# GAP-LAB-CUHK-SZ/gaustudio

Hardware: AMD Instinct MI355X
Metric: Mpixels/s fwd+bwd @1M Gaussians 1920x1080 (higher is better)
Workload: dtype f32; 1 GPU; C3: 1M synthetic Gaussians, 1920x1080, SH degree 3, fwd+bwd (colour+depth+median+opacity consumed); gaussians=1000000, width=1920, height=1080, sh_degree=3, tiles=8160, views_per_rank=1, loss=colour + depth + median + opacity gradients consumed, camera=static (the same view every step), parallelism=single GPU

## Files before the change

### __graft_entry__.py

```python
import os
import subprocess
import sys

ROOT = os.path.dirname(os.path.abspath(__file__))
if ROOT not in sys.path:
    sys.path.insert(0, ROOT)


def build() -> None:
    subprocess.check_call(["make", "-C", os.path.join(ROOT, "gaustudio_amd", "csrc"), "-j4"])
    subprocess.check_call(["make", "-C", os.path.join(ROOT, "oracle"), "all"])
    ref_script = os.path.join(ROOT, "oracle", "build_ref.sh")
    if os.path.isdir("/root/reference") and os.path.exists(ref_script):
        subprocess.check_call(["bash", ref_script])
    import ctypes
    import gaustudio_amd
    import gaustudio_diff_gaussian_rasterization as g
    L = g._C.lib()
    assert L.gsr_abi_version() == 6
    for sym in ("gsr_forward", "gsr_backward", "gsr_mark_visible", "gsr_backward_scratch_bytes", "gsr_last_error",
                "gsr_inspect_geometry", "gsr_inspect_binning", "gsr_inspect_image", "gsr_inspect_backward_sums", "gsr_set_profiling",
                "gsr_last_forward_ms", "gsr_last_backward_ms", "gsr_forward_raw", "gsr_backward_raw", "gsr_forward_ex", "gsr_backward_ex", "gsr_options_init", "gsr_depth_to_points",
                "gsr_depth_to_normals", "gsr_depth_epilogue", "gsr_backward_parts", "gsr_set_option", "gsr_get_option", "gsr_selftest", "gsr_inspect_counts", "gsr_inspect_staged", "gsr_tsdf_integrate", "gsr_tsdf_integrate_map", "gsr_tsdf_export_blocks", "gsr_tsdf_mc_classify", "gsr_tsdf_mc_emit", "gsr_msg_header_words", "gsr_visible_index", "gsr_union_index", "gsr_pack_rows", "gsr_unpack_rows", "gsr_pack_geometry", "gsr_unpack_geometry",
                "gsr_sh_grad_from_packed", "gsr_band_classes", "gsr_mesh_rasterize", "gsr_mesh_interpolate",
                "gsr_mesh_vertex_normals", "gsr_mesh_visible_faces", "gsr_psr_rasterize", "gsr_psr_spectral", "gsr_psr_interp",
                "gsr_psr_normalize", "gsr_psr_mc_classify", "gsr_psr_mc_emit", "gsr_psr_mc_normals", "gsr_psr_rasterize_bwd",
                "gsr_psr_interp_bwd", "gsr_psr_spectral_bwd", "gsr_psr_normalize_bwd", "gsr_ctsdf_touch", "gsr_ctsdf_integrate",
                "gsr_ctsdf_export_blocks", "gsr_ctsdf_mc_classify", "gsr_ctsdf_mc_emit", "gsr_hull_pack_masks", "gsr_hull_carve",
                "gsr_voxel_plan", "gsr_voxel_count", "gsr_voxel_emit", "gsr_voxel_sort", "gsr_voxel_closest",
                "gsr_mesh_bake_select", "gsr_mesh_bake_sample", "gsr_mesh_seeds",
                "gsr_mean_dist3", "gsr_mean_dist3_ex", "gsr_point_seeds", "gsr_depth_seed_pack",
                "gsr_scaffold_count", "gsr_scaffold_emit", "gsr_scaffold_backward",
                "gsr_photometric_fwd", "gsr_photometric_bwd"):
        getattr(L, sym)
    for fn in ("rasterize_gaussians", "rasterize_gaussians_backward", "mark_visible"):
        assert callable(getattr(g._C.native(), fn))
    ctypes.CDLL(os.path.join(ROOT, "oracle", "liboracle.so"))
    ctypes.CDLL(os.path.join(ROOT, "oracle", "libtsdforacle.so"))


def smoke() -> None:
    import numpy as np
    import torch
    from gaustudio_amd import scenes
    from gaustudio_diff_gaussian_rasterization import GaussianRasterizationSettings, GaussianRasterizer
    from oracle import pyoracle as po

    assert torch.cuda.is_available(), "smoke() needs a ROCm GPU"
    dev = torch.device("cuda", 0)
    cam = scenes.make_camera(256, 160)
    sc = scenes.make_scene(5000, cam, seed=0, sigma_px_median=2.0)
    leaves = {k: getattr(sc, k).to(dev).requires_grad_(True) for k in ("means3D", "scales", "rotations", "opacities", "shs")}
    means2D = torch.zeros_like(leaves["means3D"], requires_grad=True)
    rs = GaussianRasterizationSettings(cam.height, cam.width, cam.tanfovx, cam.tanfovy, torch.zeros(3), 1.0,
                                       cam.viewmatrix.to(dev), cam.projmatrix.to(dev), 3, cam.campos.to(dev), False, False)
    import gaustudio_amd
    grads = scenes.make_output_grads(cam)
    out_default = GaussianRasterizer(rs)(means3D=leaves["means3D"], means2D=means2D, opacities=leaves["opacities"], shs=leaves["shs"],
                                         scales=leaves["scales"], rotations=leaves["rotations"])
    torch.autograd.backward([out_default[0], out_default[2], out_default[3], out_default[4]], [g.to(dev) for g in grads])
    torch.cuda.synchronize()
    grads_default = {k: v.grad.clone() for k, v in leaves.items()}
    for v in leaves.values():
        v.grad = None
    with gaustudio_amd.options(fast_exp=False):
        color, radii, depth, median, opac = GaussianRasterizer(rs)(
            means3D=leaves["means3D"], means2D=means2D, opacities=leaves["opacities"], shs=leaves["shs"],
            scales=leaves["scales"], rotations=leaves["rotations"])
        torch.autograd.backward([color, depth, median, opac], [g.to(dev) for g in grads])
    torch.cuda.synchronize()

    st = po.forward(sc.means3D.numpy(), sc.opacities.numpy(), cam.viewmatrix.numpy(), cam.projmatrix.numpy(),
                    cam.campos.numpy(), cam.width, cam.height, cam.tanfovx, cam.tanfovy, sh_degree=3,
                    shs=sc.shs.numpy(), scales=sc.scales.numpy(), rotations=sc.rotations.numpy())
    bw = po.backward(st, *[g.numpy() for g in grads])
    for name, a, b in (("color", color, st["color"]), ("depth", depth, st["depth"]), ("median", median, st["median"]),
                       ("opacity", opac, st["opacity"]), ("radii", radii, st["radii"])):
        assert np.array_equal(a.detach().cpu().numpy(), b), f"smoke: {name} differs from the oracle"
    for k, ok in dict(means3D="dL_dmeans3D", scales="dL_dscales", rotations="dL_drotations", opacities="dL_dopacity",
                      shs="dL_dsh").items():
        a = leaves[k].grad.cpu().numpy()
        b = bw[ok].reshape(a.shape)
        assert np.abs(a - b).max() <= 2e-4 * np.abs(b).max(), f"smoke: grad {k} off"
    sys.path.insert(0, os.path.join(ROOT, "tests"))
    import attribution
    ours = {k: out_default[i].detach().cpu().numpy() for k, i in (("color", 0), ("depth", 2), ("opacity", 4))}
    rep = attribution.attribute_images(st, cam.width, cam.height, {k: st[k] for k in ours}, ours, tol=1e-5, depth_scale=20.0)
    assert not rep["unattributed"], f"smoke (default mode): {len(rep['unattributed'])} of {rep['flagged']} pixels beyond 1e-5 are no threshold events"
    assert np.array_equal(out_default[1].cpu().numpy(), st["radii"])
    for k, ok in dict(means3D="dL_dmeans3D", scales="dL_dscales", rotations="dL_drotations", opacities="dL_dopacity", shs="dL_dsh").items():
        a = grads_default[k].cpu().numpy()
        b = bw[ok].reshape(a.shape)
        assert np.abs(a - b).max() <= 2e-4 * np.abs(b).max(), f"smoke (default mode): grad {k} off"
    print(f"smoke ok: R={st['num_rendered']}, reproducible mode bit-exact vs oracle, default (fast_exp) mode within 1e-5 "
          f"({rep['flagged']} pixel(s) beyond it, all attributed threshold events), "
          f"5 gradient tensors within 2e-4 of scale in both")


if __name__ == "__main__":
    build()
    print("build ok")
```

### gaustudio_amd/_C.py

```python
import ctypes
import os

import torch

from . import _abi

_HERE = os.path.dirname(os.path.abspath(__file__))
_LIB_PATH = os.path.join(_HERE, "libgsrast.so")
_lib = None


def lib():
    global _lib
    if _lib is None:
        if not os.path.exists(_LIB_PATH):
            raise ImportError(
                f"{_LIB_PATH} not found: the HIP extension is not built "
                "(run `python -c 'import __graft_entry__ as g; g.build()'` or `make -C gaustudio_amd/csrc`). "
                "gaustudio_amd has no CPU fallback.")
        L = ctypes.CDLL(_LIB_PATH)
        L.gsr_last_error.restype = ctypes.c_char_p
        L.gsr_backward_scratch_bytes.restype = ctypes.c_size_t
        L.gsr_backward_scratch_bytes.argtypes = [ctypes.c_int, ctypes.c_int]
        L.gsr_abi_version.restype = ctypes.c_int
# ... 109 lines not shown


def sh_grad_from_packed(means3D, campos, msgs, offsets, degree, out):
    _call("gsr_sh_grad_from_packed", out.device, out.shape[0], int(degree), out.shape[1], offsets.numel(), means3D, campos, msgs,
          offsets, out)
    return out


def set_grad_arena(outs, keys=(), sh_chunks=1, hook=None, colors_out=None, band_split=0, band_hook=None, class_hook=None):
    native().set_grad_arena(list(outs), [int(k) for k in keys], int(sh_chunks), hook, colors_out, int(band_split), band_hook, class_hook)


def band_classes(radii, geom_buffer, split_tile_row):
    P = int(radii.shape[0])
    first = torch.empty(P, dtype=torch.int32, device=radii.device)
    second = torch.empty(P, dtype=torch.int32, device=radii.device)
    _call("gsr_band_classes", radii.device, P, radii, geom_buffer, int(split_tile_row), first, second)
    return first, second


def set_option(name, value):
    L = lib()
    rc = L.gsr_set_option(name.encode(), ctypes.c_int(int(value)))
    if rc < 0:
        raise _err(L, rc)


def get_option(name):
    return int(lib().gsr_get_option(name.encode()))


def selftest(device=None):
    dev = torch.device("cuda", torch.cuda.current_device()) if device is None else torch.device(device)
    return _call("gsr_selftest", dev)


def inspect_counts(imgBuffer, width, height):
    out = (ctypes.c_uint32 * 4)()
    _call("gsr_inspect_counts", imgBuffer.device, imgBuffer, width, height, out)
    return dict(num_binned=int(out[0]), max_tile=int(out[1]), num_rendered=int(out[2]), overflow=int(out[3]))


def inspect_staged(imgBuffer, width, height):
    out = ctypes.c_ulonglong(0)
    _call("gsr_inspect_staged", imgBuffer.device, imgBuffer, int(width), int(height), ctypes.byref(out))
    return int(out.value)


def mark_visible(means3D, viewmatrix, projmatrix):
    return native().mark_visible(means3D, viewmatrix, projmatrix)



def inspect_geometry(geomBuffer, radii):
    dev = radii.device
    P = radii.numel()
    out = dict(means2D=torch.empty((P, 2), dtype=torch.float32, device=dev),
               depths=torch.empty((P,), dtype=torch.float32, device=dev),
               conic_opacity=torch.empty((P, 4), dtype=torch.float32, device=dev),
               rgb=torch.empty((P, 3), dtype=torch.float32, device=dev),
               clamped=torch.empty((P, 3), dtype=torch.uint8, device=dev),
               tiles_touched=torch.empty((P,), dtype=torch.int32, device=dev))
    _call("gsr_inspect_geometry", dev, geomBuffer, P, radii, *out.values())
    return out


def inspect_binning(binningBuffer, imgBuffer, R, width, height):
    dev = imgBuffer.device
    T = ((width + 15) // 16) * ((height + 15) // 16)
    point_list = torch.empty((max(int(R), 0),), dtype=torch.int32, device=dev)
    ranges = torch.empty((T, 2), dtype=torch.int32, device=dev)
    _call("gsr_inspect_binning", dev, binningBuffer, imgBuffer, int(R), width, height, point_list, ranges)
    return point_list, ranges


def inspect_image(imgBuffer, width, height):
    dev = imgBuffer.device
    final_T = torch.empty((height, width), dtype=torch.float32, device=dev)
    n_contrib = torch.empty((height, width), dtype=torch.int32, device=dev)
    _call("gsr_inspect_image", dev, imgBuffer, width, height, final_T, n_contrib)
    return final_T, n_contrib


def set_profiling(enable):
    lib().gsr_set_profiling(ctypes.c_int(int(enable)))


def last_forward_ms():
    a = (ctypes.c_float * 5)()
    n = lib().gsr_last_forward_ms(a)
    if not n:
        return None
    d = dict(zip(("preprocess", "scan", "scatter", "sort", "composite"), list(a)))
    d["calls"] = n
    return d


def last_backward_ms():
    a = (ctypes.c_float * 2)()
    n = lib().gsr_last_backward_ms(a)
    if not n:
        return None
    d = dict(zip(("composite_bwd", "preprocess_bwd"), list(a)))
    d["calls"] = n
    return d
```

### gaustudio_amd/csrc/gsr_api.hip

```cpp
#include "../../include/gsrast.h"
#include "gsr_internal.h"

#include <dlfcn.h>

#include <atomic>
#include <unordered_map>
#include <cstddef>
#include <cstdio>
#include <cstdlib>
#include <cstring>
#include <mutex>
#include <string>
#include <vector>

using namespace gsr;

namespace {

thread_local std::string g_err;
struct ProfSet {
	hipEvent_t ev[6];
	uint32_t have = 0;
};
struct ProfLog {
// ... 417 lines not shown
	hipStream_t s = (hipStream_t)stream;
	g_err.clear();
	if (P <= 0) return GSR_OK;
	if (!means3D || !viewmatrix || !present) return fail(GSR_ERR_ARG, "gsr_mark_visible: NULL argument", __FILE__, __LINE__);
	const float* view = viewmatrix;
	float* tmp = nullptr;
	if (!is_device_ptr(viewmatrix)) {
		HIP_TRY(hipMallocAsync((void**)&tmp, 16 * sizeof(float), s));
		HIP_TRY(hipMemcpyAsync(tmp, viewmatrix, 16 * sizeof(float), hipMemcpyHostToDevice, s));
		view = tmp;
	}
	launch_mark_visible(P, means3D, view, present, s);
	hipError_t e = hipGetLastError();
	if (tmp) (void)hipFreeAsync(tmp, s);
	if (e != hipSuccess) return fail(GSR_ERR_HIP, "mark_visible launch", __FILE__, __LINE__, e);
	return GSR_OK;
}

static int forward_impl(const gsr_options* opt, gsr_alloc_fn geometry_alloc, void* geometry_ctx, gsr_alloc_fn binning_alloc, void* binning_ctx,
                        gsr_alloc_fn image_alloc, void* image_ctx, int P, int D, int M, const float* background,
                        int width, int height, const float* means3D, const float* shs, const float* shs_rest,
                        const float* colors_precomp, const float* opacities, const float* scales, float scale_modifier,
                        const float* rotations, const float* cov3D_precomp, int activation_flags,
                        const float* viewmatrix, const float* projmatrix, const float* cam_pos, float tan_fovx,
                        float tan_fovy, int prefiltered, float* out_color, float* out_depth, float* out_median_depth,
                        float* out_opacity, int* radii, int debug, void* stream)
{
	hipStream_t s = (hipStream_t)stream;
	g_err.clear();
	if (width <= 0 || height <= 0) return fail(GSR_ERR_ARG, "gsr_forward: bad image size", __FILE__, __LINE__);
	if (!out_color || !out_depth || !out_median_depth || !out_opacity)
		return fail(GSR_ERR_ARG, "gsr_forward: NULL output", __FILE__, __LINE__);
	const size_t HW = (size_t)width * height;
	if (P <= 0) {
		hipLaunchKernelGGL(fill_empty_outputs_kernel, dim3((unsigned)((HW + 255) / 256)), dim3(256), 0, s, HW,
		                   out_color, out_depth, out_median_depth, out_opacity);
		STAGE_CHECK("fill_empty_outputs", debug, s);
		return 0;
	}
	if (!means3D || !opacities || !viewmatrix || !projmatrix || !cam_pos || !radii)
		return fail(GSR_ERR_ARG, "gsr_forward: NULL required input", __FILE__, __LINE__);
	if (!colors_precomp && !shs)
		return fail(GSR_ERR_ARG, "For non-RGB, provide precomputed Gaussian colors!", __FILE__, __LINE__);
	if (!cov3D_precomp && (!scales || !rotations))
		return fail(GSR_ERR_ARG, "gsr_forward: need scales+rotations or cov3D_precomp", __FILE__, __LINE__);
	if (!colors_precomp && (D < 0 || D > 3 || (D + 1) * (D + 1) > M))
		return fail(GSR_ERR_ARG, "gsr_forward: SH degree does not fit the stored coefficients", __FILE__, __LINE__);
	if (!geometry_alloc || !binning_alloc || !image_alloc)
		return fail(GSR_ERR_ARG, "gsr_forward: NULL allocator", __FILE__, __LINE__);

	{
		const int rc = check_sticky("gsr_forward");
		if (rc < 0) return rc;
	}
	Resolved ro = resolve_options(opt);
#ifndef GSR_AB_VARIANTS
	if (ro.fwd_variant == 1)
		return fail(GSR_ERR_ARG, "gsr_forward: fwd_variant 1 (the per-wave A/B kernel) is not in this build (make AB=1; gsr_get_option(\"ab_variants\"))", __FILE__, __LINE__);
#endif
	if (ro.fast_exp && ro.fwd_variant == 1) {
		if (ro.fast_exp_explicit)
			return fail(GSR_ERR_ARG, "gsr_forward: fast_exp needs the per-quarter compositing kernels (fwd_variant 0)", __FILE__, __LINE__);
		ro.fast_exp = 0;
	}
	const GeomLayout gl((size_t)P);
	const ImgLayout il(width, height);
	if (il.gx > 65535 || il.gy > 65535) return fail(GSR_ERR_ARG, "gsr_forward: image too large", __FILE__, __LINE__);
	char* geom = geometry_alloc(geometry_ctx, gl.total);
	const bool lds_bin = bin_lds_path_ok(il.T);
	const size_t hm_off = il.total;
	char* img = image_alloc(image_ctx, il.total + (lds_bin ? align_up(bin_hist_bytes(P, il.T)) : 0));
	if (!geom || !img) return fail(GSR_ERR_ALLOC, "gsr_forward: allocator returned NULL", __FILE__, __LINE__);

	remember_forward_mode(img, ro.fast_exp != 0, ro.forward_only);

	GsCam* cam = reinterpret_cast<GsCam*>(geom + gl.cam);
	GsRec* recs = reinterpret_cast<GsRec*>(geom + gl.recs);
	GsCtl* ctl = reinterpret_cast<GsCtl*>(img + il.ctl);
	uint2* ranges = reinterpret_cast<uint2*>(img + il.ranges);
	uint32_t* tile_count = reinterpret_cast<uint32_t*>(img + il.tile_count);
	float* final_T = reinterpret_cast<float*>(img + il.final_T);
	uint32_t* n_contrib = reinterpret_cast<uint32_t*>(img + il.n_contrib);
	uint32_t* med_pos = reinterpret_cast<uint32_t*>(img + il.med_pos);

	Timer tm(prof_next(g_fwd_log), s, kFwdStages, g_prof_fwd_mask);
	static_assert(sizeof(GsCtl) == 8 * sizeof(uint32_t), "stage_cam_kernel clears GsCtl word by word");
	if (!lds_bin) HIP_TRY(hipMemsetAsync(img + il.ctl, 0, il.final_T - il.ctl, s));
	{
		const float* const src[4] = {viewmatrix, projmatrix, cam_pos, background};
		float* const dst[4] = {cam->view, cam->proj, cam->campos, cam->bg};
		const int n[4] = {16, 16, 3, 3};
		const bool banded = ro.band_hi > 0 || ro.band_lo > 0;
		const uint32_t word = (ro.fast_exp ? GSR_CTL_OPT_FAST_EXP : 0u) | (ro.tight ? GSR_CTL_OPT_TIGHT : 0u) |
		                      (ro.cull ? GSR_CTL_OPT_CULL : 0u) | (ro.fwd_variant == 1 ? GSR_CTL_OPT_WAVE_LISTS : 0u) |
		                      (banded ? GSR_CTL_OPT_BAND : 0u) | (ro.forward_only ? GSR_CTL_OPT_FORWARD_ONLY : 0u);
		HIP_TRY(stage_small(src, dst, n, s, &ctl->opts, word, reinterpret_cast<uint32_t*>(ctl), 8));
	}

	FwdArgs a;
	a.P = P; a.D = D; a.M = M; a.W = width; a.H = height;
	a.means3D = means3D; a.shs = shs; a.colors_precomp = colors_precomp; a.opacities = opacities;
	a.scales = scales; a.scale_modifier = scale_modifier; a.rotations = rotations; a.cov3D_precomp = cov3D_precomp;
	a.tan_fovx = tan_fovx; a.tan_fovy = tan_fovy; a.prefiltered = prefiltered;
	a.shs_rest = shs_rest; a.act = activation_flags;
	a.tight = ro.tight != 0;
	a.band_lo = ro.band_lo > 0 ? ro.band_lo : 0;
	a.band_hi = ro.band_hi;

	tm.mark();
	uint32_t* tiles_touched = reinterpret_cast<uint32_t*>(geom + gl.tiles_touched);
	uint32_t* bsums = reinterpret_cast<uint32_t*>(geom + gl.bsums);
	uint32_t* refsums = reinterpret_cast<uint32_t*>(geom + gl.refsums);
	uint32_t* Hm = reinterpret_cast<uint32_t*>(img + hm_off);
	uint4* binfo_w = reinterpret_cast<uint4*>(geom + gl.binfo);
	const uint4* binfo = (lds_bin && g_opt_bininfo.load() != 0) ? binfo_w : nullptr;
	launch_preprocess_fwd(a, cam, il, radii, recs, ro.forward_only ? nullptr : reinterpret_cast<float*>(geom + gl.shjac), binfo_w, tiles_touched, bsums, refsums,
	                      lds_bin ? nullptr : tile_count, ctl, s);
	STAGE_CHECK("preprocess_fwd", debug, s);
	tm.mark();
	if (lds_bin) {
		launch_bin_hist(P, il.gx, il.T, tiles_touched, recs, binfo, Hm, tile_count, s);
		STAGE_CHECK("bin_hist", debug, s);
	}
	GsCtl* host = pinned_ctl();
	if (!host) return fail(GSR_ERR_HIP, "hipHostMalloc", __FILE__, __LINE__);
	launch_tile_scan(il.T, tile_count, ranges, (int)gl.nblk, bsums, refsums, ctl, host, s);
	STAGE_CHECK("tile_scan", debug, s);
	hipEvent_t ev = readback_event();
	if (ev) HIP_TRY(hipEventRecord(ev, s));
	uint32_t* goff = reinterpret_cast<uint32_t*>(geom + gl.goff);
	bool goff_done = false;
	tm.mark();

	DevState& ds = dev_state();
	const bool nocull = ro.cull == 0;
	const bool wave_lists = ro.fwd_variant == 1;
	bool skew_now = g_opt_tile_order.load() != 0 && ds.skew.load() != 0;
	auto launch_rest = [&](uint32_t cap, int long_level) -> int {
		const bool with_long = long_level > 0;
		const BinLayout bl((size_t)cap, with_long, il.T);
		char* bin = binning_alloc(binning_ctx, bl.total);
		if (!bin) return fail(GSR_ERR_ALLOC, "gsr_forward: binning allocator returned NULL", __FILE__, __LINE__);
		uint64_t* keys = reinterpret_cast<uint64_t*>(bin + bl.keys);
		uint64_t* keys2 = reinterpret_cast<uint64_t*>(bin + bl.keys2);
		uint32_t* point_list = reinterpret_cast<uint32_t*>(bin + bl.point_list);
		if (cap > 0) {
			if (lds_bin) {
				launch_bin_scatter2(P, il.gx, il.T, tiles_touched, recs, binfo, Hm, ranges, keys, bsums, goff, ctl, cap, s);
				goff_done = true;
			}
			else
				launch_bin_scatter(P, il.gx, radii, tiles_touched, recs, ranges, tile_count, keys, ctl, cap, s);
			STAGE_CHECK("bin_scatter", debug, s);
		}
		if (!goff_done) {
			launch_goff_apply(P, tiles_touched, bsums, goff, s);
			STAGE_CHECK("goff_apply", debug, s);
			goff_done = true;
		}
		tm.mark();
		if (cap > 0) {
			launch_tile_sort(il.T, true, long_level, ranges, keys, keys2, point_list, bin + bl.queue, (size_t)cap, ctl, cap, long_level > 0 ? sticky_word() : nullptr, s);
			STAGE_CHECK("tile_sort", debug, s);
		}
		tm.mark();
		const uint32_t* order = nullptr;
		if (skew_now && cap > 0) {
			uint32_t* o = reinterpret_cast<uint32_t*>(img + il.tile_order);
			launch_tile_order_fwd(il.T, ranges, o, ctl, cap, s);
			order = o;
		}
		launch_composite_fwd(il, width, height, ranges, point_list, recs, out_color, out_depth, out_median_depth,
		                     out_opacity, final_T, n_contrib, med_pos, ctl, cap,
		                     long_level >= 2 ? 0xffffffffu : (long_level == 1 ? GSR_SORT_GIANT : GSR_SORT_LDS_MAX), nocull, wave_lists, ro.fast_exp != 0, order,
		                     tile_count , s);
		STAGE_CHECK("composite_fwd", debug, s);
		tm.mark();
		return 0;
	};

	const uint32_t cap0 = ds.cap.load();
	const int long0 = ds.long_lists.load();
	const bool speculate = !debug && ro.speculative != 0 && cap0 > 0;
	if (speculate) {
		const int rc = launch_rest(cap0, long0);
		if (rc < 0) return rc;
	}
	if (ev) HIP_TRY(hipEventSynchronize(ev));
	else HIP_TRY(hipStreamSynchronize(s));
	const uint32_t Rb = host->num_binned, max_tile = host->max_tile_count;
	if (host->err_prefiltered)
		return fail(GSR_ERR_PREFILTERED, "Point is filtered although prefiltered is set. This shouldn't happen!",
		            __FILE__, __LINE__);
	if ((host->err_overflow & 1u) || host->ref_rendered > 0x7fffffffu || Rb > 0x7fffffffu)
		return fail(GSR_ERR_ARG, "gsr_forward: more than 2^31 - 1 (tile, Gaussian) instances", __FILE__, __LINE__);
	const int need_long = max_tile > GSR_SORT_GIANT ? 2 : (max_tile > GSR_SORT_LDS_MAX ? 1 : 0);
	if (!speculate || Rb > cap0 || need_long > long0) {
		const int rc = launch_rest(Rb, need_long);
		if (rc < 0) return rc;
	}
	const uint32_t want = Rb + Rb / 4 + 4096u;
	uint32_t cur = ds.cap.load();
	for (;;) {
		const uint32_t next = cur < want ? want : (cur - (cur - want) / 8 > want + 4096u ? cur - (cur - want) / 8 : want);
		if (next == cur || ds.cap.compare_exchange_weak(cur, next)) break;
	}
	ds.long_lists.store(need_long);
	if (debug) {
		GsCtl c;
		HIP_TRY(hipMemcpyAsync(&c, img + il.ctl, sizeof(GsCtl), hipMemcpyDeviceToHost, s));
		HIP_TRY(hipStreamSynchronize(s));
		if (c.err_overflow & 2u)
			return fail(GSR_ERR_HIP, "gsr_forward: the long-list sort overflowed a work queue (SortQueueLayout bound violated)", __FILE__, __LINE__);
	}
	const int skew = (g_opt_tile_order.load() != 0 && max_tile > GSR_SORT_LDS_MAX && (uint64_t)max_tile * (uint64_t)il.T > 4ull * Rb) ? 1 : 0;
	remember_forward_skew(img, skew);
	ds.skew.store(skew);
	return (int)host->ref_rendered;
}

int gsr_forward(gsr_alloc_fn geometry_alloc, void* geometry_ctx, gsr_alloc_fn binning_alloc, void* binning_ctx,
                gsr_alloc_fn image_alloc, void* image_ctx, int P, int D, int M, const float* background, int width,
                int height, const float* means3D, const float* shs, const float* colors_precomp,
                const float* opacities, const float* scales, float scale_modifier, const float* rotations,
                const float* cov3D_precomp, const float* viewmatrix, const float* projmatrix, const float* cam_pos,
                float tan_fovx, float tan_fovy, int prefiltered, float* out_color, float* out_depth,
                float* out_median_depth, float* out_opacity, int* radii, int debug, void* stream)
{
	return forward_impl(nullptr, geometry_alloc, geometry_ctx, binning_alloc, binning_ctx, image_alloc, image_ctx, P, D, M,
	                    background, width, height, means3D, shs, nullptr, colors_precomp, opacities, scales,
	                    scale_modifier, rotations, cov3D_precomp, 0, viewmatrix, projmatrix, cam_pos, tan_fovx, tan_fovy,
	                    prefiltered, out_color, out_depth, out_median_depth, out_opacity, radii, debug, stream);
}

int gsr_forward_raw(gsr_alloc_fn geometry_alloc, void* geometry_ctx, gsr_alloc_fn binning_alloc, void* binning_ctx,
                    gsr_alloc_fn image_alloc, void* image_ctx, int P, int D, int M, const float* background, int width,
                    int height, const float* means3D, const float* f_dc, const float* f_rest, const float* raw_opacities,
                    const float* raw_scales, float scale_modifier, const float* raw_rotations, int activation_flags,
                    const float* viewmatrix, const float* projmatrix, const float* cam_pos, float tan_fovx,
                    float tan_fovy, int prefiltered, float* out_color, float* out_depth, float* out_median_depth,
                    float* out_opacity, int* radii, int debug, void* stream)
{
	if (P > 0 && (!f_dc || (M > 1 && !f_rest) || !raw_scales || !raw_rotations))
		return fail(GSR_ERR_ARG, "gsr_forward_raw: f_dc, f_rest, raw_scales and raw_rotations are required", __FILE__, __LINE__);
	return forward_impl(nullptr, geometry_alloc, geometry_ctx, binning_alloc, binning_ctx, image_alloc, image_ctx, P, D, M,
	                    background, width, height, means3D, f_dc, M > 1 ? f_rest : nullptr, nullptr, raw_opacities,
	                    raw_scales, scale_modifier, raw_rotations, nullptr, activation_flags, viewmatrix, projmatrix, cam_pos,
	                    tan_fovx, tan_fovy, prefiltered, out_color, out_depth, out_median_depth, out_opacity, radii, debug,
	                    stream);
}

int gsr_forward_ex(const gsr_options* opt, gsr_alloc_fn geometry_alloc, void* geometry_ctx, gsr_alloc_fn binning_alloc,
                   void* binning_ctx, gsr_alloc_fn image_alloc, void* image_ctx, int P, int D, int M,
                   const float* background, int width, int height, const float* means3D, const float* shs,
                   const float* shs_rest, const float* colors_precomp, const float* opacities, const float* scales,
                   float scale_modifier, const float* rotations, const float* cov3D_precomp, int activation_flags,
                   const float* viewmatrix, const float* projmatrix, const float* cam_pos, float tan_fovx, float tan_fovy,
                   int prefiltered, float* out_color, float* out_depth, float* out_median_depth, float* out_opacity,
                   int* radii, int debug, void* stream)
{
	return forward_impl(opt, geometry_alloc, geometry_ctx, binning_alloc, binning_ctx, image_alloc, image_ctx, P, D, M,
	                    background, width, height, means3D, shs, shs_rest, colors_precomp, opacities, scales, scale_modifier,
	                    rotations, cov3D_precomp, activation_flags, viewmatrix, projmatrix, cam_pos, tan_fovx, tan_fovy,
	                    prefiltered, out_color, out_depth, out_median_depth, out_opacity, radii, debug, stream);
}

size_t gsr_geometry_bytes(int P) { return GeomLayout((size_t)(P > 0 ? P : 0)).total; }
size_t gsr_image_bytes(int width, int height) { return (width > 0 && height > 0) ? ImgLayout(width, height).total : 0; }

size_t gsr_backward_scratch_bytes(int P, int R)
{
	return BwdLayout((size_t)(P > 0 ? P : 0), (size_t)(R > 0 ? R : 0)).total;
}

static int bwd_variant(int opt, hipStream_t s)
{
	if (opt >= 0) return opt;
	DevState& ds = dev_state();
	int st = ds.selftest.load();
	if (st < 0) {
		st = gsr_selftest((void*)s);
		if (st < 0) st = 0;
		ds.selftest.store(st);
	}
	return (st & 3) == 3 ? 0 : 1;
}

static int backward_impl(const gsr_options* opt, int parts, int sh_g0, int sh_g1, int P, int D, int M, int R, const float* background, int width, int height,
                         const float* means3D, const float* shs, const float* shs_rest, const float* colors_precomp,
                         const float* scales, float scale_modifier, const float* rotations, const float* cov3D_precomp,
                         int activation_flags, float tan_fovx, float tan_fovy, const int* radii, const char* geom_buffer,
                         const char* binning_buffer, const char* image_buffer, const float* dL_dpix,
                         const float* dL_dpix_depth, const float* dL_dpix_median_depth,
                         const float* dL_dpix_final_opacity, float* dL_dmean2D, float* dL_dopacity, float* dL_dcolor,
                         float* dL_dmean3D, float* dL_dcov3D, float* dL_dsh, float* dL_dsh_rest, float* dL_dscale,
                         float* dL_drot, char* scratch, int debug, void* stream)
{
	hipStream_t s = (hipStream_t)stream;
	g_err.clear();
	if (P <= 0) return GSR_OK;
	if (!geom_buffer || !image_buffer || !binning_buffer || !scratch || !radii || !means3D)
		return fail(GSR_ERR_ARG, "gsr_backward: NULL buffer", __FILE__, __LINE__);
	const bool sh_colors = (parts & GSR_BWD_PART_SH_COLORS) != 0;
	const int colors_early = ((parts & GSR_BWD_PART_COLORS_EARLY) && sh_colors) ? GSR_PART_COLORS_EARLY : 0;
	if (!dL_dmean2D || !dL_dopacity || !dL_dcolor || !dL_dmean3D || (!dL_dcov3D && cov3D_precomp) || !dL_dscale || !dL_drot ||
	    (M > 0 && !dL_dsh && !sh_colors))
		return fail(GSR_ERR_ARG, "gsr_backward: NULL output", __FILE__, __LINE__);
	if (sh_colors && (!shs || shs_rest || colors_precomp))
		return fail(GSR_ERR_ARG, "gsr_backward: GSR_BWD_PART_SH_COLORS needs SH colours in one [P,M,3] tensor", __FILE__, __LINE__);
	if (shs && (D < 0 || D > 3 || (D + 1) * (D + 1) > M))
		return fail(GSR_ERR_ARG, "gsr_backward: SH degree does not fit the stored coefficients", __FILE__, __LINE__);

	const GeomLayout gl((size_t)P);
	const ImgLayout il(width, height);
	const BinLayout bl((size_t)(R > 0 ? R : 0));
	const GsCam* cam = reinterpret_cast<const GsCam*>(geom_buffer + gl.cam);
	const GsRec* recs = reinterpret_cast<const GsRec*>(geom_buffer + gl.recs);
	const uint2* ranges = reinterpret_cast<const uint2*>(image_buffer + il.ranges);
	const float* final_T = reinterpret_cast<const float*>(image_buffer + il.final_T);
	const uint32_t* n_contrib = reinterpret_cast<const uint32_t*>(image_buffer + il.n_contrib);
	const uint32_t* med_pos = reinterpret_cast<const uint32_t*>(image_buffer + il.med_pos);
	const uint32_t* point_list = reinterpret_cast<const uint32_t*>(binning_buffer + bl.point_list);
	const BwdLayout wl((size_t)P, (size_t)(R > 0 ? R : 0));
	const uint32_t* goff = reinterpret_cast<const uint32_t*>(geom_buffer + gl.goff);
	const uint32_t* clampw = reinterpret_cast<const uint32_t*>(geom_buffer + gl.binfo) + 2;
	float* bg_dev = reinterpret_cast<float*>(scratch + wl.bg);
	float* rows = reinterpret_cast<float*>(scratch + wl.rows);
	uint8_t* row_flags = reinterpret_cast<uint8_t*>(scratch + wl.flags);

	const int band_phase = (parts & GSR_BWD_PART_BAND_FIRST) ? 0 : ((parts & GSR_BWD_PART_BAND_SECOND) ? 1 : -1);
	int band_split = 0;
	if (band_phase >= 0) {
		if ((parts & GSR_BWD_PART_BAND_FIRST) && (parts & GSR_BWD_PART_BAND_SECOND))
			return fail(GSR_ERR_ARG, "gsr_backward: GSR_BWD_PART_BAND_FIRST and _SECOND are two calls", __FILE__, __LINE__);
		if (!(parts & GSR_BWD_PART_MAIN) || (parts & GSR_BWD_PART_SH))
			return fail(GSR_ERR_ARG, "gsr_backward: a band call runs GSR_BWD_PART_MAIN only (the SH stage follows the second band as its own call)", __FILE__, __LINE__);
		band_split = sh_g0 < 0 ? 0 : (sh_g0 > il.gy ? il.gy : sh_g0);
	}
	BwdArgs a;
	a.cls_mode = band_phase + 1;
	a.cls_split = band_split;
	a.P = P; a.D = D; a.M = M; a.W = width; a.H = height;
	a.means3D = means3D; a.shs = shs; a.colors_precomp = colors_precomp; a.scales = scales;
	a.scale_modifier = scale_modifier; a.rotations = rotations; a.cov3D_precomp = cov3D_precomp;
	a.tan_fovx = tan_fovx; a.tan_fovy = tan_fovy; a.radii = radii;
	a.shs_rest = shs_rest; a.act = activation_flags;

	FwdMode fwd;
	{
		int rc = check_sticky("gsr_backward");
		if (rc < 0) return rc;
		rc = lookup_forward(image_buffer, il.ctl, s, &fwd);
		if (rc < 0) return rc;
	}
	if (fwd.forward_only)
		return fail(GSR_ERR_ARG, "gsr_backward: these buffers come from a forward_only forward (gsr_options.forward_only): it kept nothing for a backward", __FILE__, __LINE__);
	if (debug) {
		GsCtl c;
		HIP_TRY(hipMemcpyAsync(&c, image_buffer + il.ctl, sizeof(GsCtl), hipMemcpyDeviceToHost, s));
		HIP_TRY(hipStreamSynchronize(s));
		if (c.opts & GSR_CTL_OPT_FORWARD_ONLY)
			return fail(GSR_ERR_ARG, "gsr_backward: these buffers come from a forward_only forward (gsr_options.forward_only): it kept nothing for a backward", __FILE__, __LINE__);
		if (c.err_overflow & 2u)
			return fail(GSR_ERR_HIP, "gsr_backward: the forward's long-list sort overflowed a work queue (point_list is not sorted)", __FILE__, __LINE__);
	}
	if (!(parts & GSR_BWD_PART_MAIN)) {
		launch_preprocess_bwd(a, cam, recs, clampw, reinterpret_cast<const float*>(geom_buffer + gl.shjac), goff, rows, nullptr, dL_dmean2D, dL_dopacity, dL_dcolor, dL_dmean3D, dL_dcov3D,
		                      dL_dsh, dL_dsh_rest, dL_dscale, dL_drot, GSR_PART_SH | (sh_colors ? GSR_PART_SH_COLORS : 0) | colors_early, sh_g0, sh_g1, s);
		STAGE_CHECK("preprocess_bwd_sh", debug, s);
		return GSR_OK;
	}

	Timer tm(prof_next(g_bwd_log), s, kBwdStages, g_prof_bwd_mask);
	const bool flagged = (size_t)(R > 0 ? R : 0) > (size_t)il.T * GSR_FLAG_AVG;
	GsBg bgv;
	bgv.dptr = (background != nullptr && is_device_ptr(background)) ? background : nullptr;
	for (int i = 0; i < 3; i++) bgv.host[i] = (background != nullptr && bgv.dptr == nullptr) ? background[i] : 0.f;
	bgv.flag_dst = reinterpret_cast<uint32_t*>(bg_dev + 8);
	bgv.flag = flagged ? 1u : 0u;
	bgv.tile_order = nullptr;
	bgv.tile_lo = band_phase == 1 ? (uint32_t)band_split * (uint32_t)il.gx : 0u;
	bgv.tile_hi = band_phase == 0 ? (uint32_t)band_split * (uint32_t)il.gx : 0xffffffffu;
	if (R <= 0) {
		const float* const src[4] = {nullptr, nullptr, nullptr, nullptr};
		float* const dst[4] = {nullptr, nullptr, nullptr, nullptr};
		const int n[4] = {0, 0, 0, 0};
		HIP_TRY(stage_small(src, dst, n, s, bgv.flag_dst, bgv.flag));
	}
	if (flagged) {
		if (band_phase != 1) HIP_TRY(hipMemsetAsync(row_flags, 0, (size_t)R, s));
	} else
		row_flags = nullptr;

	tm.mark();
	if (R > 0) {
		Resolved ro = resolve_options(opt);
		{
			const int fwd_mode = fwd.fast_exp;
			if (!ro.fast_exp_explicit) ro.fast_exp = fwd_mode;
			if (fwd_mode != (ro.fast_exp != 0))
				return fail(GSR_ERR_ARG, "gsr_backward: fast_exp differs from the forward that produced these buffers", __FILE__, __LINE__);
		}
		if (debug) {
			GsCtl c;
			HIP_TRY(hipMemcpyAsync(&c, image_buffer + il.ctl, sizeof(GsCtl), hipMemcpyDeviceToHost, s));
			HIP_TRY(hipStreamSynchronize(s));
			if (!ro.fast_exp_explicit) ro.fast_exp = (c.opts & GSR_CTL_OPT_FAST_EXP) ? 1 : 0;
			if (((c.opts & GSR_CTL_OPT_FAST_EXP) != 0u) != (ro.fast_exp != 0))
				return fail(GSR_ERR_ARG, "gsr_backward: fast_exp differs from the forward that produced these buffers", __FILE__, __LINE__);
		}
		int variant = bwd_variant(ro.bwd_variant, s);
#ifndef GSR_AB_VARIANTS
		if (variant & 2)
			return fail(GSR_ERR_ARG, "gsr_backward: bwd_variant bit 1 (the per-wave A/B kernel) is not in this build (make AB=1; gsr_get_option(\"ab_variants\"))", __FILE__, __LINE__);
#endif
		if (ro.fast_exp) {
			if (variant & 2) return fail(GSR_ERR_ARG, "gsr_backward: fast_exp needs the per-quarter kernel (bwd_variant bit 1 clear)", __FILE__, __LINE__);
			variant |= 8;
		}
		if (fwd.skew) {
			uint32_t* tw = reinterpret_cast<uint32_t*>(const_cast<char*>(image_buffer) + il.tile_work);
			uint32_t* to = reinterpret_cast<uint32_t*>(const_cast<char*>(image_buffer) + il.tile_order);
			launch_tile_order(il.T, n_contrib, tw, to, s);
			bgv.tile_order = to;
		}
		launch_composite_bwd(il, width, height, bgv, ranges, point_list, recs, goff, final_T, n_contrib, med_pos, dL_dpix,
		                     dL_dpix_depth, dL_dpix_median_depth, dL_dpix_final_opacity, rows, row_flags,
		                     reinterpret_cast<const GsCtl*>(image_buffer + il.ctl), variant, s);
		STAGE_CHECK("composite_bwd", debug, s);
	}
	tm.mark();
	launch_preprocess_bwd(a, cam, recs, clampw, reinterpret_cast<const float*>(geom_buffer + gl.shjac), goff, rows, row_flags, dL_dmean2D, dL_dopacity, dL_dcolor, dL_dmean3D, dL_dcov3D, dL_dsh,
	                      dL_dsh_rest, dL_dscale, dL_drot,
	                      GSR_PART_GEOM | ((parts & GSR_BWD_PART_SH) ? GSR_PART_SH : 0) | (sh_colors ? GSR_PART_SH_COLORS : 0) | colors_early,
	                      sh_g0, sh_g1, s);
	STAGE_CHECK("preprocess_bwd", debug, s);
	tm.mark();
	return GSR_OK;
}

int gsr_backward(int P, int D, int M, int R, const float* background, int width, int height, const float* means3D,
                 const float* shs, const float* colors_precomp, const float* scales, float scale_modifier,
                 const float* rotations, const float* cov3D_precomp, const float* viewmatrix,
                 const float* projmatrix, const float* campos, float tan_fovx, float tan_fovy, const int* radii,
                 const char* geom_buffer, const char* binning_buffer, const char* image_buffer,
                 const float* dL_dpix, const float* dL_dpix_depth, const float* dL_dpix_median_depth,
                 const float* dL_dpix_final_opacity, float* dL_dmean2D, float* dL_dopacity, float* dL_dcolor,
                 float* dL_dmean3D, float* dL_dcov3D, float* dL_dsh, float* dL_dscale, float* dL_drot,
                 char* scratch, int debug, void* stream)
{
	(void)viewmatrix; (void)projmatrix; (void)campos;
	return backward_impl(nullptr, GSR_BWD_PART_MAIN | GSR_BWD_PART_SH, 0, P, P, D, M, R, background, width, height, means3D, shs, nullptr, colors_precomp, scales,
	                     scale_modifier, rotations, cov3D_precomp, 0, tan_fovx, tan_fovy, radii, geom_buffer,
	                     binning_buffer, image_buffer, dL_dpix, dL_dpix_depth, dL_dpix_median_depth,
	                     dL_dpix_final_opacity, dL_dmean2D, dL_dopacity, dL_dcolor, dL_dmean3D, dL_dcov3D, dL_dsh,
	                     nullptr, dL_dscale, dL_drot, scratch, debug, stream);
}

int gsr_backward_parts(int parts, int sh_g0, int sh_g1, int P, int D, int M, int R, const float* background, int width,
                       int height, const float* means3D, const float* shs, const float* colors_precomp, const float* scales,
                       float scale_modifier, const float* rotations, const float* cov3D_precomp, float tan_fovx,
                       float tan_fovy, const int* radii, const char* geom_buffer, const char* binning_buffer,
                       const char* image_buffer, const float* dL_dpix, const float* dL_dpix_depth,
                       const float* dL_dpix_median_depth, const float* dL_dpix_final_opacity, float* dL_dmean2D,
                       float* dL_dopacity, float* dL_dcolor, float* dL_dmean3D, float* dL_dcov3D, float* dL_dsh,
                       float* dL_dscale, float* dL_drot, char* scratch, int debug, void* stream)
{
	if (!(parts & (GSR_BWD_PART_MAIN | GSR_BWD_PART_SH)))
		return fail(GSR_ERR_ARG, "gsr_backward_parts: nothing to do", __FILE__, __LINE__);
	if ((parts & GSR_BWD_PART_SH) && sh_g0 % 256 != 0)
		return fail(GSR_ERR_ARG, "gsr_backward_parts: sh_g0 must be a multiple of 256", __FILE__, __LINE__);
	return backward_impl(nullptr, parts, sh_g0, sh_g1, P, D, M, R, background, width, height, means3D, shs, nullptr, colors_precomp,
	                     scales, scale_modifier, rotations, cov3D_precomp, 0, tan_fovx, tan_fovy, radii, geom_buffer,
	                     binning_buffer, image_buffer, dL_dpix, dL_dpix_depth, dL_dpix_median_depth,
	                     dL_dpix_final_opacity, dL_dmean2D, dL_dopacity, dL_dcolor, dL_dmean3D, dL_dcov3D, dL_dsh,
	                     nullptr, dL_dscale, dL_drot, scratch, debug, stream);
}

int gsr_backward_ex(const gsr_options* opt, int parts, int sh_g0, int sh_g1, int P, int D, int M, int R,
                    const float* background, int width, int height, const float* means3D, const float* shs,
                    const float* shs_rest, const float* colors_precomp, const float* scales, float scale_modifier,
                    const float* rotations, const float* cov3D_precomp, int activation_flags, float tan_fovx,
                    float tan_fovy, const int* radii, const char* geom_buffer, const char* binning_buffer,
                    const char* image_buffer, const float* dL_dpix, const float* dL_dpix_depth,
                    const float* dL_dpix_median_depth, const float* dL_dpix_final_opacity, float* dL_dmean2D,
                    float* dL_dopacity, float* dL_dcolor, float* dL_dmean3D, float* dL_dcov3D, float* dL_dsh,
                    float* dL_dsh_rest, float* dL_dscale, float* dL_drot, char* scratch, int debug, void* stream)
{
	if (!(parts & (GSR_BWD_PART_MAIN | GSR_BWD_PART_SH)))
		return fail(GSR_ERR_ARG, "gsr_backward_ex: nothing to do", __FILE__, __LINE__);
	if ((parts & GSR_BWD_PART_SH) && !(parts & (GSR_BWD_PART_BAND_FIRST | GSR_BWD_PART_BAND_SECOND)) && sh_g0 % 256 != 0)
		return fail(GSR_ERR_ARG, "gsr_backward_ex: sh_g0 must be a multiple of 256", __FILE__, __LINE__);
	return backward_impl(opt, parts, sh_g0, sh_g1, P, D, M, R, background, width, height, means3D, shs, shs_rest,
	                     colors_precomp, scales, scale_modifier, rotations, cov3D_precomp, activation_flags, tan_fovx, tan_fovy,
	                     radii, geom_buffer, binning_buffer, image_buffer, dL_dpix, dL_dpix_depth, dL_dpix_median_depth,
	                     dL_dpix_final_opacity, dL_dmean2D, dL_dopacity, dL_dcolor, dL_dmean3D, dL_dcov3D, dL_dsh, dL_dsh_rest,
	                     dL_dscale, dL_drot, scratch, debug, stream);
}

int gsr_band_classes(int P, const int* radii, const char* geom_buffer, int split_tile_row, int* first, int* second, void* stream)
{
	g_err.clear();
	if (P <= 0) return GSR_OK;
	if (!radii || !geom_buffer) return fail(GSR_ERR_ARG, "gsr_band_classes: NULL argument", __FILE__, __LINE__);
	const GeomLayout gl((size_t)P);
	launch_band_classes(P, radii, reinterpret_cast<const GsRec*>(geom_buffer + gl.recs), split_tile_row, first, second, (hipStream_t)stream);
	STAGE_CHECK("band_classes", 0, (hipStream_t)stream);
	return GSR_OK;
}
// ... 134 lines not shown
int gsr_backward_raw(int P, int D, int M, int R, const float* background, int width, int height, const float* means3D,
                     const float* f_dc, const float* f_rest, const float* raw_scales, float scale_modifier,
                     const float* raw_rotations, int activation_flags, float tan_fovx, float tan_fovy,
                     const int* radii, const char* geom_buffer, const char* binning_buffer, const char* image_buffer,
                     const float* dL_dpix, const float* dL_dpix_depth, const float* dL_dpix_median_depth,
                     const float* dL_dpix_final_opacity, float* dL_dmean2D, float* dL_draw_opacity, float* dL_dcolor,
                     float* dL_dmean3D, float* dL_dcov3D, float* dL_df_dc, float* dL_df_rest, float* dL_draw_scale,
                     float* dL_draw_rot, char* scratch, int debug, void* stream)
{
	if (P > 0 && (!f_dc || (M > 1 && (!f_rest || !dL_df_rest)) || !dL_df_dc))
		return fail(GSR_ERR_ARG, "gsr_backward_raw: f_dc / f_rest and their gradient outputs are required", __FILE__, __LINE__);
	return backward_impl(nullptr, GSR_BWD_PART_MAIN | GSR_BWD_PART_SH, 0, P, P, D, M, R, background, width, height, means3D, f_dc, M > 1 ? f_rest : nullptr, nullptr, raw_scales,
	                     scale_modifier, raw_rotations, nullptr, activation_flags, tan_fovx, tan_fovy, radii, geom_buffer,
	                     binning_buffer, image_buffer, dL_dpix, dL_dpix_depth, dL_dpix_median_depth,
	                     dL_dpix_final_opacity, dL_dmean2D, dL_draw_opacity, dL_dcolor, dL_dmean3D, dL_dcov3D, dL_df_dc,
	                     M > 1 ? dL_df_rest : nullptr, dL_draw_scale, dL_draw_rot, scratch, debug, stream);
}

int gsr_inspect_geometry(const char* geom_buffer, int P, const int* radii, float* means2D, float* depths,
                         float* conic_opacity, float* rgb, unsigned char* clamped, uint32_t* tiles_touched,
                         void* stream)
{
	hipStream_t s = (hipStream_t)stream;
	g_err.clear();
	if (P <= 0) return GSR_OK;
	if (!geom_buffer || !radii) return fail(GSR_ERR_ARG, "gsr_inspect_geometry: NULL buffer", __FILE__, __LINE__);
	const GeomLayout gl((size_t)P);
	hipLaunchKernelGGL(inspect_geometry_kernel, dim3((P + 255) / 256), dim3(256), 0, s, P, radii,
	                   reinterpret_cast<const GsRec*>(geom_buffer + gl.recs),
	                   reinterpret_cast<const uint32_t*>(geom_buffer + gl.tiles_touched), means2D, depths, conic_opacity, rgb,
	                   clamped, tiles_touched);
	STAGE_CHECK("inspect_geometry", 0, s);
	return GSR_OK;
}

int gsr_inspect_backward_sums(const char* geom_buffer, const char* scratch, int P, int R, const int* radii,
                               float* sums, void* stream)
{
	hipStream_t s = (hipStream_t)stream;
	g_err.clear();
	if (P <= 0) return GSR_OK;
	if (!geom_buffer || !scratch || !radii || !sums)
		return fail(GSR_ERR_ARG, "gsr_inspect_backward_sums: NULL argument", __FILE__, __LINE__);
	const GeomLayout gl((size_t)P);
	const BwdLayout wl((size_t)P, (size_t)(R > 0 ? R : 0));
	uint32_t flagged = 0;
	HIP_TRY(hipMemcpyAsync(&flagged, scratch + wl.bg + 8 * sizeof(float), sizeof(uint32_t), hipMemcpyDeviceToHost, s));
	HIP_TRY(hipStreamSynchronize(s));
	launch_inspect_sums(P, radii, reinterpret_cast<const GsRec*>(geom_buffer + gl.recs),
	                    reinterpret_cast<const uint32_t*>(geom_buffer + gl.goff),
	                    reinterpret_cast<const float*>(scratch + wl.rows), flagged ? reinterpret_cast<const uint8_t*>(scratch + wl.flags) : nullptr,
	                    sums, s);
	STAGE_CHECK("inspect_backward_sums", 0, s);
	return GSR_OK;
}

int gsr_inspect_binning(const char* binning_buffer, const char* image_buffer, int R, int width, int height,
                        uint32_t* point_list, uint32_t* ranges, void* stream)
{
	hipStream_t s = (hipStream_t)stream;
	g_err.clear();
	if (!image_buffer) return fail(GSR_ERR_ARG, "gsr_inspect_binning: NULL buffer", __FILE__, __LINE__);
	const ImgLayout il(width, height);
	const BinLayout bl((size_t)(R > 0 ? R : 0));
	if (ranges) HIP_TRY(hipMemcpyAsync(ranges, image_buffer + il.ranges, sizeof(uint2) * (size_t)il.T, hipMemcpyDeviceToDevice, s));
	if (point_list && R > 0) {
		if (!binning_buffer) return fail(GSR_ERR_ARG, "gsr_inspect_binning: NULL binning buffer", __FILE__, __LINE__);
		HIP_TRY(hipMemcpyAsync(point_list, binning_buffer + bl.point_list, sizeof(uint32_t) * (size_t)R, hipMemcpyDeviceToDevice, s));
	}
	return GSR_OK;
}

int gsr_inspect_image(const char* image_buffer, int width, int height, float* final_T, uint32_t* n_contrib,
                      void* stream)
{
	hipStream_t s = (hipStream_t)stream;
	g_err.clear();
	if (!image_buffer) return fail(GSR_ERR_ARG, "gsr_inspect_image: NULL buffer", __FILE__, __LINE__);
	const ImgLayout il(width, height);
	hipLaunchKernelGGL(inspect_image_kernel, dim3(il.T), dim3(256), 0, s, il.gx, width, height,
	                   reinterpret_cast<const float*>(image_buffer + il.final_T),
	                   reinterpret_cast<const uint32_t*>(image_buffer + il.n_contrib), final_T, n_contrib);
	STAGE_CHECK("inspect_image", 0, s);
	return GSR_OK;
}

int gsr_surfel_forward(const gsr_options* opt, gsr_alloc_fn geometry_alloc, void* geometry_ctx, gsr_alloc_fn binning_alloc,
                       void* binning_ctx, gsr_alloc_fn image_alloc, void* image_ctx, int P, int D, int M, const float* background,
                       int width, int height, const float* means3D, const float* shs, const float* colors_precomp,
                       const float* opacities, const float* scales, float scale_modifier, const float* rotations,
                       const float* viewmatrix, const float* projmatrix, const float* cam_pos, float* out_color, float* out_allmap,
                       int* radii, int debug, void* stream)
{
	hipStream_t s = (hipStream_t)stream;
	g_err.clear();
	if (width <= 0 || height <= 0) return fail(GSR_ERR_ARG, "gsr_surfel_forward: bad image size", __FILE__, __LINE__);
	if (!out_color || !out_allmap) return fail(GSR_ERR_ARG, "gsr_surfel_forward: NULL output", __FILE__, __LINE__);
	if (!geometry_alloc || !binning_alloc || !image_alloc)
		return fail(GSR_ERR_ARG, "gsr_surfel_forward: NULL allocator", __FILE__, __LINE__);
	const size_t HW = (size_t)width * height;
	if (P <= 0) {
		HIP_TRY(hipMemsetAsync(out_color, 0, sizeof(float) * 3 * HW, s));
		HIP_TRY(hipMemsetAsync(out_allmap, 0, sizeof(float) * 7 * HW, s));
		return 0;
	}
	if (!means3D || !opacities || !scales || !rotations || !viewmatrix || !projmatrix || !cam_pos || !radii)
		return fail(GSR_ERR_ARG, "gsr_surfel_forward: NULL required input", __FILE__, __LINE__);
	if ((colors_precomp != nullptr) == (shs != nullptr))
		return fail(GSR_ERR_ARG, "gsr_surfel_forward: provide exactly one of SHs or precomputed colours", __FILE__, __LINE__);
	if (!colors_precomp && (D < 0 || D > 3 || (D + 1) * (D + 1) > M))
		return fail(GSR_ERR_ARG, "gsr_surfel_forward: SH degree does not fit the stored coefficients", __FILE__, __LINE__);
	{
		const int rc = check_sticky("gsr_surfel_forward");
		if (rc < 0) return rc;
	}
	const Resolved ro = resolve_options(opt);
	const SurfGeomLayout gl((size_t)P);
	const ImgLayout il0(width, height);
	if (!bin_lds_path_ok(il0.T))
		return fail(GSR_ERR_ARG, "gsr_surfel_forward: image too large (the surfel path bins through the LDS tile histogram only)", __FILE__, __LINE__);
	const SurfImgLayout sl(width, height, bin_hist_bytes(P, il0.T));
	const ImgLayout& il = sl.il;
	char* geom = geometry_alloc(geometry_ctx, gl.total);
	char* img = image_alloc(image_ctx, sl.total);
	if (!geom || !img) return fail(GSR_ERR_ALLOC, "gsr_surfel_forward: allocator returned NULL", __FILE__, __LINE__);
	remember_forward_mode(img, ro.fast_exp != 0, 0);

	GsCam* cam = reinterpret_cast<GsCam*>(geom + gl.cam);
	SurfRec* recs = reinterpret_cast<SurfRec*>(geom + gl.recs);
	uint32_t* tiles_touched = reinterpret_cast<uint32_t*>(geom + gl.tiles_touched);
	uint32_t* goff = reinterpret_cast<uint32_t*>(geom + gl.goff);
	uint32_t* bsums = reinterpret_cast<uint32_t*>(geom + gl.bsums);
	uint32_t* refsums = reinterpret_cast<uint32_t*>(geom + gl.refsums);
	uint4* binfo = reinterpret_cast<uint4*>(geom + gl.binfo);
	GsCtl* ctl = reinterpret_cast<GsCtl*>(img + il.ctl);
	uint2* ranges = reinterpret_cast<uint2*>(img + il.ranges);
	uint32_t* tile_count = reinterpret_cast<uint32_t*>(img + il.tile_count);
	uint32_t* Hm = reinterpret_cast<uint32_t*>(img + sl.hist);
	{
		const float* const src[4] = {viewmatrix, projmatrix, cam_pos, background};
		float* const dst[4] = {cam->view, cam->proj, cam->campos, cam->bg};
		const int n[4] = {16, 16, 3, 3};
		HIP_TRY(stage_small(src, dst, n, s, &ctl->opts, ro.fast_exp ? GSR_CTL_OPT_FAST_EXP : 0u, reinterpret_cast<uint32_t*>(ctl), 8));
	}
	SurfFwdArgs a;
	a.P = P; a.D = D; a.M = M; a.W = width; a.H = height;
	a.means3D = means3D; a.shs = shs; a.colors_precomp = colors_precomp; a.opacities = opacities;
	a.scales = scales; a.scale_modifier = scale_modifier; a.rotations = rotations;
	launch_surfel_preprocess_fwd(a, cam, il, radii, recs, reinterpret_cast<float*>(geom + gl.shjac), binfo, tiles_touched, bsums, refsums, s);
	STAGE_CHECK("surfel_preprocess_fwd", debug, s);
	launch_bin_hist(P, il.gx, il.T, tiles_touched, nullptr, binfo, Hm, tile_count, s);
	STAGE_CHECK("bin_hist", debug, s);
	GsCtl* host = pinned_ctl();
	if (!host) return fail(GSR_ERR_HIP, "hipHostMalloc", __FILE__, __LINE__);
	launch_tile_scan(il.T, tile_count, ranges, (int)gl.nblk, bsums, refsums, ctl, host, s);
	STAGE_CHECK("tile_scan", debug, s);
	hipEvent_t ev = readback_event();
	if (ev) {
		HIP_TRY(hipEventRecord(ev, s));
		HIP_TRY(hipEventSynchronize(ev));
	} else
		HIP_TRY(hipStreamSynchronize(s));
	const uint32_t R = host->num_binned, max_tile = host->max_tile_count;
	if ((host->err_overflow & 1u) || host->ref_rendered > 0x7fffffffu || R > 0x7fffffffu)
		return fail(GSR_ERR_ARG, "gsr_surfel_forward: more than 2^31 - 1 (tile, surfel) instances", __FILE__, __LINE__);
	const int long_level = max_tile > GSR_SORT_GIANT ? 2 : (max_tile > GSR_SORT_LDS_MAX ? 1 : 0);
// ... 95 lines not shown
```

### gaustudio_amd/csrc/gsr_internal.h

```cpp
#pragma once
#include "gsr_common.h"
#include <stddef.h>

namespace gsr {

static inline size_t align_up(size_t v, size_t a = 256) { return (v + a - 1) / a * a; }

#define GSR_PRE_BLOCK 256
struct GeomLayout {
	size_t cam, recs, tiles_touched, goff, bsums, refsums, shjac, binfo, total;
	size_t nblk;
	explicit GeomLayout(size_t P)
	{
		nblk = (P + GSR_PRE_BLOCK - 1) / GSR_PRE_BLOCK;
		cam = 0;
		recs = align_up(sizeof(GsCam));
		tiles_touched = recs + align_up(sizeof(GsRec) * P);
		goff = tiles_touched + align_up(sizeof(uint32_t) * P);
		bsums = goff + align_up(sizeof(uint32_t) * (P + 1));
		refsums = bsums + align_up(sizeof(uint32_t) * (nblk + 1));
		shjac = refsums + align_up(sizeof(uint32_t) * (nblk + 1));
		binfo = shjac + align_up(sizeof(float) * 9 * P);
		total = binfo + align_up(sizeof(uint4) * P);
	}
};

struct ImgLayout {
	size_t ctl, ranges, tile_count, final_T, n_contrib, med_pos, tile_work, tile_order, total;
	int gx, gy, T;
	ImgLayout(int W, int H)
	{
		gx = (W + GSR_BLOCK_X - 1) / GSR_BLOCK_X;
		gy = (H + GSR_BLOCK_Y - 1) / GSR_BLOCK_Y;
		T = gx * gy;
		ctl = 0;
		ranges = align_up(sizeof(GsCtl));
		tile_count = ranges + align_up(sizeof(uint2) * (size_t)T);
		final_T = tile_count + align_up(sizeof(uint32_t) * (size_t)T);
		n_contrib = final_T + align_up(sizeof(float) * (size_t)T * GSR_TILE_PIX);
		med_pos = n_contrib + align_up(sizeof(uint32_t) * (size_t)T * GSR_TILE_PIX);
		tile_work = med_pos + align_up(sizeof(uint32_t) * (size_t)T * GSR_TILE_PIX);
		tile_order = tile_work + align_up(sizeof(uint32_t) * (size_t)T);
		total = tile_order + align_up(sizeof(uint32_t) * (size_t)T);
	}
};

size_t sort_queue_bytes(size_t R, int T);
struct BinLayout {
	size_t point_list, keys, keys2, queue, total;
	explicit BinLayout(size_t R, bool with_tmp = false, int T = 0)
	{
		point_list = 0;
		keys = align_up(sizeof(uint32_t) * R);
		keys2 = keys + align_up(sizeof(uint64_t) * R);
		queue = keys2 + align_up(sizeof(uint64_t) * R);
		total = with_tmp ? queue + align_up(sort_queue_bytes(R, T)) : keys2;
		if (total == 0) total = 256;
	}
};
#define GSR_SORT_LDS_MAX 1024u

struct FwdArgs {
	int P, D, M, W, H;
	const float* means3D;
	const float* shs;
	const float* colors_precomp;
	const float* opacities;
	const float* scales;
	float scale_modifier;
	const float* rotations;
	const float* cov3D_precomp;
	float tan_fovx, tan_fovy;
	int prefiltered;
	const float* shs_rest;
	int act;
	int tight;
	int band_lo, band_hi;
};

void launch_mark_visible(int P, const float* means3D, const float* view, unsigned char* present, hipStream_t s);
void launch_preprocess_fwd(const FwdArgs& a, const GsCam* cam, const ImgLayout& il, int* radii, GsRec* recs, float* shjac, uint4* binfo,
                           uint32_t* tiles_touched, uint32_t* bsums, uint32_t* refsums, uint32_t* tile_count,
                           GsCtl* ctl, hipStream_t s);
void launch_tile_scan(int T, uint32_t* tile_count, uint2* ranges, int nblk, uint32_t* bsums, const uint32_t* refsums,
                      GsCtl* ctl, GsCtl* host_ctl, hipStream_t s);
void launch_goff_apply(int P, const uint32_t* tiles_touched, const uint32_t* bsums, uint32_t* goff, hipStream_t s);
void launch_bin_scatter(int P, int gx, const int* radii, const uint32_t* tiles_touched, const GsRec* recs,
                        const uint2* ranges, uint32_t* cursor, uint64_t* keys, const GsCtl* ctl, uint32_t cap,
                        hipStream_t s);
int bin_chunks(int P, int T);
size_t bin_hist_bytes(int P, int T);
bool bin_lds_path_ok(int T);
void launch_bin_hist(int P, int gx, int T, const uint32_t* tiles_touched, const GsRec* recs, const uint4* binfo, uint32_t* Hm,
                     uint32_t* tile_count, hipStream_t s);
void launch_bin_scatter2(int P, int gx, int T, const uint32_t* tiles_touched, const GsRec* recs, const uint4* binfo, uint32_t* Hm,
                         const uint2* ranges, uint64_t* keys, const uint32_t* bsums, uint32_t* goff, const GsCtl* ctl, uint32_t cap, hipStream_t s);
#define GSR_PART_REGS 8192u
#define GSR_SORT_MANY 1024u
#ifndef GSR_SORT_GIANT
#define GSR_SORT_GIANT 8192u
#endif
void launch_tile_sort(int T, bool with_short, int long_level, const uint2* ranges, uint64_t* keys, uint64_t* keys2,
                      uint32_t* point_list, char* queue, size_t R, GsCtl* ctl, uint32_t cap, uint32_t* host_err, hipStream_t s);
void launch_composite_fwd(const ImgLayout& il, int W, int H, const uint2* ranges, const uint32_t* point_list,
                          const GsRec* recs, float* out_color, float* out_depth, float* out_median,
                          float* out_opacity, float* final_T, uint32_t* n_contrib, uint32_t* med_pos, GsCtl* ctl, uint32_t cap, uint32_t max_sorted, bool nocull, bool wave_lists, bool fast_exp,
                          const uint32_t* tile_order, uint32_t* staged_out, hipStream_t s);
void launch_tile_order_fwd(int T, const uint2* ranges, uint32_t* order, const GsCtl* ctl, uint32_t cap, hipStream_t s);

struct BwdArgs {
	int P, D, M, W, H;
	const float* means3D;
	const float* shs;
	const float* colors_precomp;
	const float* scales;
	float scale_modifier;
	const float* rotations;
	const float* cov3D_precomp;
	float tan_fovx, tan_fovy;
	const int* radii;
	const float* shs_rest;
	int act;
	int cls_mode = 0, cls_split = 0;
};
#define GSR_ROW_STRIDE 12
#define GSR_FLAG_AVG 1024
#ifndef GSR_SUM_SLAB
#define GSR_SUM_SLAB 96
#endif
struct BwdLayout {
	size_t bg, flags, rows, total;
	BwdLayout(size_t P, size_t R)
	{
		(void)P;
		bg = 0;
		flags = bg + 256;
		rows = flags + align_up(R > 0 ? R : 1);
		total = rows + align_up(sizeof(float) * GSR_ROW_STRIDE * (R > 0 ? R : 1));
	}
};
struct GsBg {
	const float* dptr;
	float host[3];
	uint32_t* flag_dst;
	uint32_t flag;
	const uint32_t* tile_order;
	uint32_t tile_lo, tile_hi;
};
void launch_band_classes(int P, const int* radii, const GsRec* recs, int split, int* first, int* second, hipStream_t s);
void launch_tile_order(int T, const uint32_t* n_contrib, uint32_t* tile_work, uint32_t* tile_order, hipStream_t s);
void launch_composite_bwd(const ImgLayout& il, int W, int H, const GsBg& bg, const uint2* ranges,
                          const uint32_t* point_list, const GsRec* recs, const uint32_t* goff, const float* final_T,
                          const uint32_t* n_contrib, const uint32_t* med_pos, const float* dL_dpix, const float* dL_dpix_depth,
                          const float* dL_dpix_median, const float* dL_dpix_opacity, float* rows, uint8_t* row_flags,
                          const GsCtl* ctl, int variant, hipStream_t s);
#define GSR_PART_GEOM 1
#define GSR_PART_SH 2
#define GSR_PART_SH_COLORS 4
#define GSR_PART_COLORS_EARLY 8
void launch_preprocess_bwd(const BwdArgs& a, const GsCam* cam, const GsRec* recs, const uint32_t* clampw, const float* shjac, const uint32_t* goff,
                           const float* rows, const uint8_t* row_flags, float* dL_dmean2D, float* dL_dopacity, float* dL_dcolor,
                           float* dL_dmean3D, float* dL_dcov3D, float* dL_dsh, float* dL_dsh_rest, float* dL_dscale,
                           float* dL_drot, int parts, int sh_g0, int sh_g1, hipStream_t s);
void launch_bwd_selftest(const float* in, uint32_t* out, hipStream_t s);
void launch_sh_grad_from_colors(int P, int D, int M, int N, const float* means3D, const float* campos, const float* colors,
                                const uint32_t* msgs, const unsigned long long* msg_off, uint32_t hdr_words, float* dL_dsh, hipStream_t s);
void launch_inspect_sums(int P, const int* radii, const GsRec* recs, const uint32_t* goff, const float* rows,
                         const uint8_t* row_flags,
                         float* sums10, hipStream_t s);

struct __attribute__((aligned(16))) SurfRec {
	float4 q0, q1, q2, q3, q4;
};
static_assert(sizeof(SurfRec) == 80, "SurfRec must be 80 bytes");
struct SurfGeomLayout {
	size_t cam, recs, tiles_touched, goff, bsums, refsums, shjac, binfo, total;
	size_t nblk;
	explicit SurfGeomLayout(size_t P)
	{
		nblk = (P + GSR_PRE_BLOCK - 1) / GSR_PRE_BLOCK;
		cam = 0;
		recs = align_up(sizeof(GsCam));
		tiles_touched = recs + align_up(sizeof(SurfRec) * P);
		goff = tiles_touched + align_up(sizeof(uint32_t) * P);
		bsums = goff + align_up(sizeof(uint32_t) * (P + 1));
		refsums = bsums + align_up(sizeof(uint32_t) * (nblk + 1));
		shjac = refsums + align_up(sizeof(uint32_t) * (nblk + 1));
		binfo = shjac + align_up(sizeof(float) * 9 * P);
		total = binfo + align_up(sizeof(uint4) * P);
	}
};
struct SurfImgLayout {
	ImgLayout il;
	size_t m1, m2, m0, hist, total;
	SurfImgLayout(int W, int H, size_t hist_bytes) : il(W, H)
	{
		m1 = il.total;
		m2 = m1 + align_up(sizeof(float) * (size_t)il.T * GSR_TILE_PIX);
		m0 = m2 + align_up(sizeof(float) * (size_t)il.T * GSR_TILE_PIX);
		hist = m0 + align_up(sizeof(float) * (size_t)il.T * GSR_TILE_PIX);
		total = hist + align_up(hist_bytes > 0 ? hist_bytes : 1);
	}
};
#define GSR_SURF_ROW 16
struct SurfFwdArgs {
	int P, D, M, W, H;
	const float* means3D;
	const float* shs;
	const float* colors_precomp;
	const float* opacities;
	const float* scales;
	float scale_modifier;
	const float* rotations;
};
void launch_surfel_preprocess_fwd(const SurfFwdArgs& a, const GsCam* cam, const ImgLayout& il, int* radii, SurfRec* recs, float* shjac,
                                  uint4* binfo, uint32_t* tiles_touched, uint32_t* bsums, uint32_t* refsums, hipStream_t s);
void launch_surfel_composite_fwd(const ImgLayout& il, int W, int H, const uint2* ranges, const uint32_t* point_list, const SurfRec* recs,
                                 const GsCam* cam, float* out_color, float* out_allmap, float* final_T, uint32_t* n_contrib,
                                 uint32_t* med_pos, float* m1, float* m2, float* m0, bool fast_exp, hipStream_t s);
void launch_surfel_composite_bwd(const ImgLayout& il, int W, int H, const uint2* ranges, const uint32_t* point_list, const SurfRec* recs,
                                 const uint4* binfo, const uint32_t* goff, const float* final_T,
                                 const uint32_t* n_contrib, const uint32_t* med_pos, const float* m1, const float* m2, const float* m0,
                                 const GsCam* cam, const float* dL_dcolor, const float* dL_dallmap,
                                 float* rows, bool fast_exp, hipStream_t s);
void launch_surfel_preprocess_bwd(int P, int W, int H, const float* means3D, const float* scales, float scale_modifier,
                                  const float* rotations, const int* radii, const GsCam* cam, const SurfRec* recs,
                                  const uint32_t* goff, const float* rows, float* dL_dmean2D, float* dL_dopacity, float* dL_dcolor,
                                  float* dL_dmean3D, float* dL_dscale, float* dL_drot, hipStream_t s);

}
```

### gaustudio_amd/csrc/gsr_kernels_bwd.hip

```cpp
#include "gsr_internal.h"
#include "gsr_bwd_timing.h"

namespace gsr {

__device__ __constant__ float bSH_C0 = 0.28209479177387814f;
__device__ __constant__ float bSH_C1 = 0.4886025119029199f;
__device__ __constant__ float bSH_C2[5] = {1.0925484305920792f, -1.0925484305920792f, 0.31539156525252005f,
                                            -1.0925484305920792f, 0.5462742152960396f};
__device__ __constant__ float bSH_C3[7] = {-0.5900435899266435f, 2.890611442640554f, -0.4570457994644658f,
                                            0.3731763325901154f, -0.4570457994644658f, 1.445305721320277f,
                                            -0.5900435899266435f};

#define GSR_DPP_ADD(v, ctrl) v += __int_as_float(__builtin_amdgcn_update_dpp(0, __float_as_int(v), ctrl, 0xF, 0xF, true))
#define GSR_DPP_OF(v, ctrl) __int_as_float(__builtin_amdgcn_update_dpp(0, __float_as_int(v), ctrl, 0xF, 0xF, true))
__device__ __forceinline__ float half_swap_sum(float a, float b)
{
	const auto t = __builtin_amdgcn_permlane32_swap(__float_as_uint(a), __float_as_uint(b), false, false);
	return __uint_as_float(t[0]) + __uint_as_float(t[1]);
}
__device__ __forceinline__ float row_swap_sum(float p, float q)
{
	const auto t = __builtin_amdgcn_permlane16_swap(__float_as_uint(p), __float_as_uint(q), false, false);
	return __uint_as_float(t[0]) + __uint_as_float(t[1]);
}
// ... 55 lines not shown
			a_[0] += v0.x; a_[1] += v0.y; a_[2] += v0.z; a_[3] += v0.w; a_[4] += v1.x; a_[5] += v1.y;
			a_[6] += v1.z; a_[7] += v1.w; a_[8] += v2.x; a_[9] += v2.y;
		}
	}
	gs_sum_long_rows(b, e, rows, row_flags, lane, a_);
	if (idx >= P) return;
#pragma unroll
	for (int i = 0; i < 10; i++) out[10 * (size_t)idx + i] = a_[i];
}

void launch_inspect_sums(int P, const int* radii, const GsRec* recs, const uint32_t* goff, const float* rows,
                         const uint8_t* row_flags, float* sums10, hipStream_t s)
{
	hipLaunchKernelGGL(inspect_sums_kernel, dim3((P + 255) / 256), dim3(256), 0, s, P, radii, recs, goff, rows, row_flags,
	                   sums10);
}

#define GSR_BWD_THREADS 256
#define GSR_BWD_BATCH 64
#ifndef GSR_BWD_UNITS
#define GSR_BWD_UNITS 8
#endif
#define GSR_SLAB_STRIDE 65
#define GSR_PLANE_STRIDE 10
#define GSR_TAB_ROW 17

#ifdef GSR_AB_VARIANTS
__device__ __forceinline__ void gs_bwd_phase2(const int n, const float2* __restrict__ slab, const unsigned long long unit_js,
                                              const float4* __restrict__ sA, const float4* __restrict__ tab, const float fbx,
                                              const float fby, const int top, float* __restrict__ plane, const int lane)
{
	constexpr int NG = 64 / GSR_BWD_UNITS;
	constexpr int PPL = GSR_BWD_UNITS;
	const int u = lane & (GSR_BWD_UNITS - 1), g = lane / GSR_BWD_UNITS;
	const bool act = u < n;
	const int j = act ? (int)((unit_js >> (8 * u)) & 0xffull) : 0;
	const float2 ctr = *reinterpret_cast<const float2*>(&sA[j]);
	const uint32_t pos1 = (uint32_t)(top - j);
	const int prow = NG == 8 ? g : (g >> 1), pcol0 = NG == 8 ? 0 : ((g & 1) << 2);
	const float dy = ctr.y - (fby + (float)prow);
	const float X = ctr.x - (fbx + (float)pcol0);
	const float2* row = slab + u * GSR_SLAB_STRIDE + prow * 8 + pcol0;
	const float4* trow = tab + prow * GSR_TAB_ROW + 2 * pcol0;
	float S0 = 0.f, a0 = 0.f, a2 = 0.f, a5 = 0.f, a6 = 0.f, a7 = 0.f, a8 = 0.f, a9 = 0.f;
#pragma unroll
	for (int sx = 0; sx < PPL; sx++) {
		const float2 v = row[sx];
		const float4 c0 = trow[2 * sx], c1 = trow[2 * sx + 1];
		const float dx = X - (float)sx;
		const float t = v.x * dx;
		S0 += v.x;
		a0 += t;
		a2 = FMA(t, dx, a2);
		a5 = FMA(v.y, c1.x, a5);
		a6 = FMA(v.y, c0.x, a6);
		a7 = FMA(v.y, c0.y, a7);
		a8 = FMA(v.y, c0.z, a8);
		a9 = FMA(v.y, c0.w, a9) + ((__float_as_uint(c1.z) == pos1) ? c1.y : 0.f);
	}
	a5 += S0;
	const float a1 = dy * S0, a3 = dy * a0, a4 = dy * a1;
	const float r0 = half_swap_sum(a0, a1);
	const float r1 = half_swap_sum(a2, a3);
	const float r2 = half_swap_sum(a4, a5);
	const float r3 = half_swap_sum(a6, a7);
	const float r4 = half_swap_sum(a8, a9);
	float s0 = row_swap_sum(r0, r1), s1 = row_swap_sum(r2, r3), s2 = row_swap_sum(r4, 0.f);
	GSR_DPP_ADD(s0, 0x128); GSR_DPP_ADD(s1, 0x128); GSR_DPP_ADD(s2, 0x128);
	if (NG == 16) { GSR_DPP_ADD(s0, 0x124); GSR_DPP_ADD(s1, 0x124); GSR_DPP_ADD(s2, 0x124); }
	if (act && (lane & (16 - GSR_BWD_UNITS) & 15) == 0) {
		const int rw = lane >> 4;
		float* dst = plane + j * GSR_PLANE_STRIDE + (((rw & 1) << 1) | (rw >> 1));
		dst[0] = s0;
		dst[4] = s1;
		if ((rw & 1) == 0) dst[8] = s2;
	}
}

template <bool FLAGS, bool TSEL>
__global__ __launch_bounds__(GSR_BWD_THREADS) void composite_bwd_kernel(
    int T, int chunk, int gx, int W, int H, const GsBg bgv, const uint2* __restrict__ ranges,
    const uint32_t* __restrict__ point_list, const GsRec* __restrict__ recs, const uint32_t* __restrict__ goff,
    const float* __restrict__ final_T, const uint32_t* __restrict__ n_contrib, const uint32_t* __restrict__ med_pos,
    const float* __restrict__ dL_dpix, const float* __restrict__ dL_dpix_depth, const float* __restrict__ dL_dpix_median,
    const float* __restrict__ dL_dpix_opacity, float* __restrict__ rows, uint8_t* __restrict__ row_flags,
    const GsCtl* __restrict__ ctl)
{
	__shared__ float4 sA[GSR_BWD_BATCH];
	__shared__ float4 sB[GSR_BWD_BATCH];
	__shared__ float4 sC[GSR_BWD_BATCH];
	__shared__ uint32_t s_row[GSR_BWD_BATCH];
	__shared__ __attribute__((aligned(16))) float s_plane[4][GSR_BWD_BATCH * GSR_PLANE_STRIDE];
	__shared__ float2 s_slab[4][GSR_BWD_UNITS * GSR_SLAB_STRIDE];
	__shared__ float4 s_tab[4][8 * GSR_TAB_ROW];
	__shared__ int s_max[4];
	if (blockIdx.x == 0 && threadIdx.x == 0 && bgv.flag_dst != nullptr) *bgv.flag_dst = bgv.flag;
	const int tb_lo = (int)bgv.tile_lo, tb_n = (int)min(bgv.tile_hi, (uint32_t)T) - tb_lo;
	const int local = (blockIdx.x & 7) * chunk + (blockIdx.x >> 3);
	const int tile = bgv.tile_order ? ((int)blockIdx.x < T ? (int)bgv.tile_order[blockIdx.x] : T) : tb_lo + local;
	if ((!bgv.tile_order && ((int)(blockIdx.x >> 3) >= chunk || local >= tb_n)) || tile >= T) return;
	if ((uint32_t)tile < bgv.tile_lo || (uint32_t)tile >= bgv.tile_hi) return;
	const int tid = threadIdx.x;
	const int lane = tid & 63, wv = tid >> 6;
	const int tx = tile % gx, ty = tile / gx;
	int lx, ly;
	gs_pixel_of_thread(tid, lx, ly);
	const int px = tx * GSR_BLOCK_X + lx, py = ty * GSR_BLOCK_Y + ly;
	const bool inside = px < W && py < H;
	const float pixfx = (float)px, pixfy = (float)py;
	const float fbx = (float)(tx * GSR_BLOCK_X + ((wv & 1) << 3)), fby = (float)(ty * GSR_BLOCK_Y + ((wv >> 1) << 3));
	const float bx1 = fminf(fbx + 7.f, (float)(W - 1)), by1 = fminf(fby + 7.f, (float)(H - 1));
	const uint2 range = ranges[tile];

	const size_t sidx = (size_t)tile * GSR_TILE_PIX + tid;
	const float T_final = inside ? final_T[sidx] : 0.f;
	const int lc = inside ? (int)n_contrib[sidx] : 0;
	float dLp0 = 0.f, dLp1 = 0.f, dLp2 = 0.f, dLd = 0.f, dLo = 0.f;
	{
		float dLm = 0.f;
		uint32_t mpos = 0u;
		if (inside) {
			const size_t HW = (size_t)H * W;
			const size_t pix_id = (size_t)W * py + px;
			if (dL_dpix) {
				dLp0 = dL_dpix[pix_id];
				dLp1 = dL_dpix[HW + pix_id];
				dLp2 = dL_dpix[2 * HW + pix_id];
			}
			if (dL_dpix_depth) dLd = dL_dpix_depth[pix_id];
			if (dL_dpix_median) dLm = dL_dpix_median[pix_id];
			if (dL_dpix_opacity) dLo = dL_dpix_opacity[pix_id];
			mpos = med_pos[sidx];
		}
		float4* t = s_tab[wv] + (lane >> 3) * GSR_TAB_ROW + 2 * (lane & 7);
		t[0] = make_float4(dLp0, dLp1, dLp2, dLd);
		t[1] = make_float4(dLo, dLm, __uint_as_float(mpos), 0.f);
	}
	const float bg0 = bgv.dptr ? bgv.dptr[0] : bgv.host[0], bg1 = bgv.dptr ? bgv.dptr[1] : bgv.host[1], bg2 = bgv.dptr ? bgv.dptr[2] : bgv.host[2];
	const float bg_dot = FMA(bg2, dLp2, FMA(bg1, dLp1, FMA(bg0, dLp0, 0.f)));
	const bool any_bg = __ballot(bg_dot != 0.f) != 0ull;
	float T_ = T_final;
	float S = 0.f;

	int wmax = lc;
#pragma unroll
	for (int o = 32; o > 0; o >>= 1) wmax = max(wmax, __shfl_xor(wmax, o, 64));
	wmax = __builtin_amdgcn_readfirstlane(wmax);
	if (lane == 0) s_max[wv] = wmax;
	__syncthreads();
	const int bmax = max(max(s_max[0], s_max[1]), max(s_max[2], s_max[3]));

	for (int i = bmax + tid; !FLAGS && i < (int)(range.y - range.x); i += GSR_BWD_THREADS) {
		const uint32_t id = point_list[range.x + i];
		const uint4 q3 = recs[id].q3;
		float4* dst = reinterpret_cast<float4*>(rows + (size_t)(goff[id] + gs_row_in_rect(q3.x, q3.y, (q3.z >> GSR_Q3Z_DEAD_SHIFT) & 15u, tx, ty)) * GSR_ROW_STRIDE);
		dst[0] = make_float4(0.f, 0.f, 0.f, 0.f);
		dst[1] = make_float4(0.f, 0.f, 0.f, 0.f);
		dst[2] = make_float4(0.f, 0.f, 0.f, 0.f);
	}
	float2* slab = s_slab[wv];
	float* plane = s_plane[wv];
	const int srec = tid >> 2, spart = tid & 3;
	auto load_id = [&](int t) -> uint32_t {
		return (t > 0 && srec < min(GSR_BWD_BATCH, t)) ? point_list[range.x + (uint32_t)(t - 1 - srec)] : 0u;
	};
	auto load_part = [&](int t, uint32_t id) -> float4 {
		float4 v = make_float4(0.f, 0.f, 0.f, 0.f);
// ... 55 lines not shown
			nu++;
			if (nu == GSR_BWD_UNITS) {
				__builtin_amdgcn_fence(__ATOMIC_RELEASE, "wavefront");
				__builtin_amdgcn_wave_barrier();
				gs_bwd_phase2(GSR_BWD_UNITS, slab, unit_js, sA, s_tab[wv], fbx, fby, top, plane, lane);
				__builtin_amdgcn_wave_barrier();
				nu = 0;
				unit_js = 0ull;
			}
		};
		if (m) {
			int j0 = __ffsll((long long)m) - 1, j1 = 0;
			m &= m - 1;
			float4 A0 = sA[j0], B0 = sB[j0], C0 = sC[j0], A1, B1, C1;
			while (true) {
				const bool more1 = m != 0ull;
				if (more1) {
					j1 = __ffsll((long long)m) - 1;
					m &= m - 1;
					A1 = sA[j1]; B1 = sB[j1]; C1 = sC[j1];
				}
				pair(A0, B0, C0, j0);
				if (!more1) break;
				const bool more0 = m != 0ull;
				if (more0) {
					j0 = __ffsll((long long)m) - 1;
					m &= m - 1;
					A0 = sA[j0]; B0 = sB[j0]; C0 = sC[j0];
				}
				pair(A1, B1, C1, j1);
				if (!more0) break;
			}
		}
		if (nu > 0) {
			__builtin_amdgcn_fence(__ATOMIC_RELEASE, "wavefront");
			__builtin_amdgcn_wave_barrier();
			gs_bwd_phase2(nu, slab, unit_js, sA, s_tab[wv], fbx, fby, top, plane, lane);
		}
		__syncthreads();
		if (tid < cnt) {
			float v[10];
#pragma unroll
			for (int k = 0; k < 10; k++)
				v[k] = ((s_plane[0][tid * GSR_PLANE_STRIDE + k] + s_plane[1][tid * GSR_PLANE_STRIDE + k]) +
				        s_plane[2][tid * GSR_PLANE_STRIDE + k]) + s_plane[3][tid * GSR_PLANE_STRIDE + k];
			const float4 A = sA[tid], B = sB[tid];
			const float ca = -2.f * A.z, cb = -A.w, cc = -2.f * B.x, op = B.y;
			const float M10 = v[0], M01 = v[1], M20 = v[2], M11 = v[3], M02 = v[4];
			const float ddelx_dx = (float)(0.5 * W), ddely_dy = (float)(0.5 * H);
			const uint32_t my_row = s_row[tid];
			float4* dst = reinterpret_cast<float4*>(rows + (size_t)my_row * GSR_ROW_STRIDE);
			dst[0] = make_float4(-(op * FMA(cb, M01, ca * M10)) * ddelx_dx, -(op * FMA(cb, M10, cc * M01)) * ddely_dy,
			                     -0.5f * op * M20, -0.5f * op * M11);
			dst[1] = make_float4(-0.5f * op * M02, v[5], v[6], v[7]);
			dst[2] = make_float4(v[8], v[9], 0.f, 0.f);
			if (FLAGS) row_flags[my_row] = 1;
		}
		part_cur = part_next;
	}
}

#endif

#define GSR_BWQ_U 4
#ifndef GSR_BWQ_BATCH
#define GSR_BWQ_BATCH 128
#endif
#define GSR_BWQ_HALVES ((GSR_BWQ_BATCH + 63) / 64)
#define GSR_BWQ_LIST (GSR_BWQ_BATCH + 8)
#define GSR_BWQ_SENT GSR_BWQ_BATCH
#define GSR_BWQ_ENTRY(j) ((uint32_t)(j) << 4)
template <bool B> struct GsBool { static constexpr bool value = B; };
#define GSR_WAIT_VM0() __builtin_amdgcn_s_waitcnt(0x0F70)
#define GSR_BWQ_QSTRIDE 66

#ifndef GSR_BWQ_WAVES
#define GSR_BWQ_WAVES 4
#endif
template <bool FLAGS, bool TSEL, bool FX, bool CONLY>
__global__ __launch_bounds__(GSR_BWD_THREADS) __attribute__((amdgpu_waves_per_eu(GSR_BWQ_WAVES, GSR_BWQ_WAVES))) void composite_bwd_quarter_kernel(
    int T, int chunk, int gx, int W, int H, const GsBg bgv, const uint2* __restrict__ ranges,
    const uint32_t* __restrict__ point_list, const GsRec* __restrict__ recs, const uint32_t* __restrict__ goff,
    const float* __restrict__ final_T, const uint32_t* __restrict__ n_contrib, const uint32_t* __restrict__ med_pos,
    const float* __restrict__ dL_dpix, const float* __restrict__ dL_dpix_depth, const float* __restrict__ dL_dpix_median,
    const float* __restrict__ dL_dpix_opacity, float* __restrict__ rows, uint8_t* __restrict__ row_flags,
    const GsCtl* __restrict__ ctl)
{
	__shared__ float4 sA[GSR_BWQ_BATCH + 1];
	__shared__ float4 sB[GSR_BWQ_BATCH + 1];
	__shared__ float4 sC[GSR_BWQ_BATCH + 1];
	__shared__ uint32_t s_row[GSR_BWQ_BATCH];
	__shared__ uint16_t s_qmask[GSR_BWQ_BATCH];
	__shared__ __attribute__((aligned(16))) float s_plane[4][GSR_BWQ_BATCH * GSR_PLANE_STRIDE];
	__shared__ __attribute__((aligned(16))) float2 s_slab[4][4 * GSR_BWQ_QSTRIDE];
	__shared__ __attribute__((aligned(16))) uint16_t s_list[4][4][GSR_BWQ_LIST];
	__shared__ int s_max[4];
	if (blockIdx.x == 0 && threadIdx.x == 0 && bgv.flag_dst != nullptr) *bgv.flag_dst = bgv.flag;
	const int tb_lo = (int)bgv.tile_lo, tb_n = (int)min(bgv.tile_hi, (uint32_t)T) - tb_lo;
	const int local = (blockIdx.x & 7) * chunk + (blockIdx.x >> 3);
	const int tile = bgv.tile_order ? ((int)blockIdx.x < T ? (int)bgv.tile_order[blockIdx.x] : T) : tb_lo + local;
	if ((!bgv.tile_order && ((int)(blockIdx.x >> 3) >= chunk || local >= tb_n)) || tile >= T) return;
	if ((uint32_t)tile < bgv.tile_lo || (uint32_t)tile >= bgv.tile_hi) return;
	const int tid = threadIdx.x;
	const int lane = tid & 63, wv = __builtin_amdgcn_readfirstlane(tid >> 6), qd = lane >> 4;
	TM_DECL
	const int tx = tile % gx, ty = tile / gx;
	const int lx = ((wv & 1) << 3) + ((qd & 1) << 2) + (lane & 3);
	const int ly = ((wv >> 1) << 3) + ((qd >> 1) << 2) + ((lane >> 2) & 3);
	const int px = tx * GSR_BLOCK_X + lx, py = ty * GSR_BLOCK_Y + ly;
	const bool inside = px < W && py < H;
	const float pixfx = (float)px, pixfy = (float)py;
	const float fbx = (float)(tx * GSR_BLOCK_X + ((wv & 1) << 3)), fby = (float)(ty * GSR_BLOCK_Y + ((wv >> 1) << 3));
	const uint2 range = ranges[tile];
	const bool have_qmask = __builtin_amdgcn_readfirstlane(ctl->has_qmask) != 0u;
	const uint16_t* __restrict__ qmask = gs_qmask_ptr(point_list, __builtin_amdgcn_readfirstlane(ctl->num_binned));

	const size_t sidx = (size_t)tile * GSR_TILE_PIX + (wv << 6) + ((ly & 7) << 3) + (lx & 7);
	const float T_final = inside ? final_T[sidx] : 0.f;
	const int lc = inside ? (int)n_contrib[sidx] : 0;
	float dLp0 = 0.f, dLp1 = 0.f, dLp2 = 0.f, dLd = 0.f, dLo = 0.f, dLm = 0.f;
	uint32_t mpos = 0u;
	if (inside) {
		const size_t HW = (size_t)H * W;
		const size_t pix_id = (size_t)W * py + px;
		if (dL_dpix) {
			dLp0 = dL_dpix[pix_id];
			dLp1 = dL_dpix[HW + pix_id];
			dLp2 = dL_dpix[2 * HW + pix_id];
		}
		if (!CONLY) {
			if (dL_dpix_depth) dLd = dL_dpix_depth[pix_id];
			if (dL_dpix_median) dLm = dL_dpix_median[pix_id];
			if (dL_dpix_opacity) dLo = dL_dpix_opacity[pix_id];
			mpos = med_pos[sidx];
		}
	}
	float2* slab = s_slab[wv];
	float* plane = s_plane[wv];
	const int u2 = (lane >> 2) & 3, r2 = lane & 3;
	float4 g_pix[4];
	float g_op[4];
	{
		float4* tmp = reinterpret_cast<float4*>(slab);
		tmp[2 * lane] = make_float4(dLp0, dLp1, dLp2, dLd);
		if (!CONLY) tmp[2 * lane + 1] = make_float4(dLo, 0.f, 0.f, 0.f);
		__builtin_amdgcn_fence(__ATOMIC_RELEASE, "wavefront");
		__builtin_amdgcn_wave_barrier();
#pragma unroll
		for (int sx = 0; sx < 4; sx++) {
			const int pl = (qd << 4) + (r2 << 2) + sx;
			const float4 gp = tmp[2 * pl];
			const float c0 = gp.x, c1 = gp.y, c2 = gp.z, c3 = gp.w;
			g_pix[sx] = make_float4(r2 == 0 ? c0 : r2 == 1 ? c1 : r2 == 2 ? c2 : c3, r2 == 0 ? c1 : r2 == 1 ? c0 : r2 == 2 ? c3 : c2,
			                        r2 == 0 ? c2 : r2 == 1 ? c3 : r2 == 2 ? c0 : c1, r2 == 0 ? c3 : r2 == 1 ? c2 : r2 == 2 ? c1 : c0);
			g_op[sx] = CONLY ? 0.f : tmp[2 * pl + 1].x;
		}
		__builtin_amdgcn_wave_barrier();
#pragma unroll
		for (int sx = 0; sx < 4; sx++) asm volatile("" : "+v"(g_pix[sx].x), "+v"(g_pix[sx].y), "+v"(g_pix[sx].z), "+v"(g_pix[sx].w));
	}
	const float y2 = fby + (float)(((qd >> 1) << 2) + r2), x2 = fbx + (float)((qd & 1) << 2);
	const float bg0 = bgv.dptr ? bgv.dptr[0] : bgv.host[0], bg1 = bgv.dptr ? bgv.dptr[1] : bgv.host[1], bg2 = bgv.dptr ? bgv.dptr[2] : bgv.host[2];
	const float bg_dot = FMA(bg2, dLp2, FMA(bg1, dLp1, FMA(bg0, dLp0, 0.f)));
	const bool any_bg = __ballot(bg_dot != 0.f) != 0ull;
	float T_ = T_final;
	float S = 0.f;

	int qmax = lc;
	qmax = max(qmax, __shfl_xor(qmax, 1, 64));
	qmax = max(qmax, __shfl_xor(qmax, 2, 64));
	qmax = max(qmax, __shfl_xor(qmax, 4, 64));
	qmax = max(qmax, __shfl_xor(qmax, 8, 64));
	const int qm0 = __builtin_amdgcn_readlane(qmax, 0), qm1 = __builtin_amdgcn_readlane(qmax, 16);
	const int qm2 = __builtin_amdgcn_readlane(qmax, 32), qm3 = __builtin_amdgcn_readlane(qmax, 48);
	const int wmax = max(max(qm0, qm1), max(qm2, qm3));
	if (lane == 0) s_max[wv] = wmax;
	TM(0)
	if (tid < 3) (tid == 0 ? sA : tid == 1 ? sB : sC)[GSR_BWQ_SENT] = make_float4(0.f, 0.f, 0.f, 0.f);
	__syncthreads();
	const int bmax = max(max(s_max[0], s_max[1]), max(s_max[2], s_max[3]));
	TM(1)

	const int srec = tid >> 2, spart = tid & 3;
	const uint32_t* __restrict__ tile_list = point_list + range.x;
	const uint32_t* __restrict__ mask_words = have_qmask ? reinterpret_cast<const uint32_t*>(qmask) : point_list;
	auto list_pos = [&](int t, int h) -> uint32_t {
		return (uint32_t)max(t - 1 - (srec + 64 * h), 0);
	};
	auto word_ptr = [&](int t, int h, uint32_t id) -> const uint32_t* {
		return spart == 2 ? mask_words + ((range.x + list_pos(t, h)) >> 1) : goff + id;
	};
	uint32_t id_next[GSR_BWQ_HALVES];
	float4 part[GSR_BWQ_HALVES];
#pragma unroll
	for (int h = 0; h < GSR_BWQ_HALVES; h++) {
		part[h] = make_float4(0.f, 0.f, 0.f, 0.f);
		id_next[h] = 0u;
	}
	if (bmax > 0) {
		uint32_t id_cur[GSR_BWQ_HALVES];
#pragma unroll
		for (int h = 0; h < GSR_BWQ_HALVES; h++) {
			id_cur[h] = tile_list[list_pos(bmax, h)];
			id_next[h] = tile_list[list_pos(bmax - GSR_BWQ_BATCH, h)];
		}
#pragma unroll
		for (int h = 0; h < GSR_BWQ_HALVES; h++) {
			part[h] = reinterpret_cast<const float4*>(recs + id_cur[h])[spart];
			if (spart >= 2) part[h].w = __uint_as_float(*word_ptr(bmax, h, id_cur[h]));
		}
	}
	for (int i = bmax + tid; !FLAGS && i < (int)(range.y - range.x); i += GSR_BWD_THREADS) {
		const uint32_t id = tile_list[i];
		const uint4 q3 = recs[id].q3;
		float4* dst = reinterpret_cast<float4*>(rows + (size_t)(goff[id] + gs_row_in_rect(q3.x, q3.y, (q3.z >> GSR_Q3Z_DEAD_SHIFT) & 15u, tx, ty)) * GSR_ROW_STRIDE);
		dst[0] = make_float4(0.f, 0.f, 0.f, 0.f);
		dst[1] = make_float4(0.f, 0.f, 0.f, 0.f);
		dst[2] = make_float4(0.f, 0.f, 0.f, 0.f);
	}
	GSR_WAIT_VM0();
	TM(2)
	const uint16_t* my_list = &s_list[wv][qd][0];
	int thr16 = (bmax - 1 - lc) * 16;
	const char* recA = reinterpret_cast<const char*>(sA);
	const char* recB = reinterpret_cast<const char*>(sB);
	const char* recC = reinterpret_cast<const char*>(sC);
	float2* my_slab_w = slab + qd * GSR_BWQ_QSTRIDE + (lane & 15);
	const float4* my_slab_r = reinterpret_cast<const float4*>(slab + qd * GSR_BWQ_QSTRIDE + u2 * 16 + r2 * 4);

	for (int top = bmax; top > 0; top -= GSR_BWQ_BATCH) {
		const int cnt = min(GSR_BWQ_BATCH, top);
		TM(3)
		__syncthreads();
		TM(4)
#pragma unroll
		for (int h = 0; h < GSR_BWQ_HALVES; h++) {
			const int sr = srec + 64 * h;
			if (sr < cnt) {
				if (spart == 0) sA[sr] = part[h];
				else if (spart == 1) {
					float* b = reinterpret_cast<float*>(&sB[sr]);
					*reinterpret_cast<float2*>(b) = make_float2(part[h].x, part[h].y);
					b[2] = part[h].z;
					reinterpret_cast<float2*>(&sC[sr])[1] = make_float2(part[h].w, 0.f);
				} else if (spart == 2) {
					reinterpret_cast<float*>(&sB[sr])[3] = part[h].x;
					*reinterpret_cast<float2*>(&sC[sr]) = make_float2(part[h].y, part[h].z);
					s_qmask[sr] = (uint16_t)(__float_as_uint(part[h].w) >> (16u * ((range.x + (uint32_t)(top - 1 - sr)) & 1u)));
				} else {
					const uint32_t q3x = __float_as_uint(part[h].x), q3y = __float_as_uint(part[h].y), q3z = __float_as_uint(part[h].z);
					s_row[sr] = __float_as_uint(part[h].w) + gs_row_in_rect(q3x, q3y, (q3z >> GSR_Q3Z_DEAD_SHIFT) & 15u, tx, ty);
				}
			}
		}
		TM(5)
#pragma unroll
		for (int h = 0; h < GSR_BWQ_HALVES; h++) {
			part[h] = reinterpret_cast<const float4*>(recs + id_next[h])[spart];
			if (spart >= 2) part[h].w = __uint_as_float(*word_ptr(top - GSR_BWQ_BATCH, h, id_next[h]));
		}
#pragma unroll
		for (int h = 0; h < GSR_BWQ_HALVES; h++) id_next[h] = tile_list[list_pos(top - 2 * GSR_BWQ_BATCH, h)];
		float zero = 0.f;
		uint32_t ss = GSR_BWQ_ENTRY(GSR_BWQ_SENT) * 0x00010001u;
		asm volatile("" : "+v"(zero), "+v"(ss));
		for (int i = tid; i < 4 * GSR_BWQ_BATCH * GSR_PLANE_STRIDE / 4; i += GSR_BWD_THREADS)
			reinterpret_cast<float4*>(&s_plane[0][0])[i] = make_float4(zero, zero, zero, zero);
		static_assert((4 * GSR_BWQ_LIST * sizeof(uint16_t)) % 16 == 0, "a wave's lists are filled 16 B at a time");
		for (int i = lane; i < (int)(4 * GSR_BWQ_LIST * sizeof(uint16_t) / 16); i += 64)
			reinterpret_cast<uint4*>(&s_list[wv][0][0])[i] = make_uint4(ss, ss, ss, ss);
		TM(6)
		__syncthreads();
		TM(7)
		if (mpos != 0u && dLm != 0.f && (uint32_t)top >= mpos && (uint32_t)top - mpos < (uint32_t)cnt)
			atomicAdd(&plane[((uint32_t)top - mpos) * GSR_PLANE_STRIDE + 7], dLm);
		int c0 = 0, c1 = 0, c2 = 0, c3 = 0;
#define GSR_APPEND(QQ, CNT)                                                                                          \
	{                                                                                                                \
		const bool h_ = (mk >> (QQ)) & 1u;                                                                           \
		const unsigned long long bm = __ballot(h_);                                                                  \
		const int pos_ = CNT + (int)__builtin_amdgcn_mbcnt_hi((uint32_t)(bm >> 32), __builtin_amdgcn_mbcnt_lo((uint32_t)bm, 0u)); \
		if (h_) s_list[wv][QQ][pos_] = (uint16_t)GSR_BWQ_ENTRY(jl);                                                  \
		CNT += __popcll(bm);                                                                                         \
	}
#pragma unroll
		for (int h = 0; h < GSR_BWQ_HALVES; h++) {
			const int jl = lane + 64 * h;
			if (64 * h >= cnt) break;
			uint32_t mk = 0;
			if (jl < cnt) {
				if (have_qmask) {
					const uint32_t m16 = (uint32_t)s_qmask[jl] >> (8 * (wv >> 1) + 2 * (wv & 1));
					mk = (m16 & 3u) | ((m16 >> 2) & 12u);
				} else {
					float4 q1 = sB[jl];
					q1.w = sC[jl].z;
					mk = gs_quarter_mask<2>(sA[jl], q1, fbx, fby, 0xfu);
				}
				const int pos = top - 1 - jl;
				mk &= (pos < qm0 ? 1u : 0u) | (pos < qm1 ? 2u : 0u) | (pos < qm2 ? 4u : 0u) | (pos < qm3 ? 8u : 0u);
			}
			GSR_APPEND(0, c0)
			GSR_APPEND(1, c1)
			GSR_APPEND(2, c2)
			GSR_APPEND(3, c3)
		}
#undef GSR_APPEND
		__builtin_amdgcn_wave_barrier();
		TM(8)
		const int n = max(max(c0, c1), max(c2, c3));
		const int my_cnt = qd == 0 ? c0 : qd == 1 ? c1 : qd == 2 ? c2 : c3;
		struct Rec { float4 A, B; float2 C; float pcut; };
		auto fetch = [&](const uint32_t e) -> Rec {
			Rec r;
			r.A = *reinterpret_cast<const float4*>(recA + e);
			r.B = *reinterpret_cast<const float4*>(recB + e);
			if (FX) {
				r.C = *reinterpret_cast<const float2*>(recC + e);
				r.pcut = 0.f;
			} else {
				float4 c = *reinterpret_cast<const float4*>(recC + e);
				asm volatile("" : "+v"(c.w));
				r.C = make_float2(c.x, c.y);
				r.pcut = c.z;
			}
			return r;
		};
		auto step = [&](const Rec& rc, const uint32_t e, const int st, auto BG) {
			const float4 A = rc.A, B = rc.B;
			const float3 Cc = make_float3(B.w, rc.C.x, rc.C.y);
			const bool in_front = (int)e > thr16;
			const float dx = A.x - pixfx, dy = A.y - pixfy;
			const float power = FMA(A.w * dx, dy, FMA(B.x * dy, dy, (A.z * dx) * dx));
			float G, a0;
			bool live;
			if (!FX) {
				G = gs_exp(power);
				a0 = B.y * G;
				live = in_front & (power <= 0.0f) & (power >= rc.pcut) & (!(a0 < 1.0f / 255.0f));
			} else {
				G = gs_exp_hw(power);
				a0 = B.y * G;
				live = in_front & (power <= 0.0f) & (!(a0 < 1.0f / 255.0f));
			}
			const float Gm = live ? G : 0.f;
			const float alpha = fminf(0.99f, B.y * Gm);
			const float rinv = __builtin_amdgcn_rcpf(1.0f - alpha);
			const float test_T = T_ * rinv;
			const float w = alpha * test_T;
			const float cd = FMA(Cc.x, dLp0, FMA(Cc.y, dLp1, FMA(Cc.z, dLp2, CONLY ? 0.f : FMA(B.z, dLd, dLo))));
			const float diff = cd - S;
			float dL_dalpha = diff * test_T;
			if (decltype(BG)::value) dL_dalpha = FMA(-(T_final * rinv), bg_dot, dL_dalpha);
			const float q = Gm * dL_dalpha;
			S = FMA(alpha, diff, S);
			T_ = TSEL ? (live ? test_T : T_) : test_T;
			my_slab_w[16 * st] = make_float2(q, w);
		};
		float pn0 = 0.f, pn1 = 0.f, pn2 = 0.f, t0 = 0.f, t1 = 0.f, t2 = 0.f;
		float* pn_dst = plane;
		bool pn_act = false;
		const bool r2_hi = (r2 & 2) != 0;
		auto turn_read = [&](const int qq) {
			if (pn_act & (qd == qq)) {
				t0 = pn_dst[0];
				t1 = pn_dst[4];
				if (!r2_hi) t2 = pn_dst[8];
			}
		};
		auto turn_write = [&](const int qq) {
			if (pn_act & (qd == qq)) {
				pn_dst[0] = t0 + pn0;
				pn_dst[4] = t1 + pn1;
				if (!r2_hi) pn_dst[8] = t2 + pn2;
			}
		};
		const uint32_t sel2 = 0x0c0c0000u | ((2u * u2 + 1u) << 8) | (2u * u2);
		auto phase2 = [&](const uint2 cur, const int i) {
			{
				const bool act = i + u2 < my_cnt;
// ... 43 lines not shown
			turn_read(1); step(fetch(cur.x >> 16), cur.x >> 16, 1, BG); turn_write(1);                                      \
			turn_read(2); step(fetch(cur.y & 0xffffu), cur.y & 0xffffu, 2, BG); turn_write(2);                              \
			turn_read(3); step(fetch(cur.y >> 16), cur.y >> 16, 3, BG); turn_write(3);                                      \
			__builtin_amdgcn_fence(__ATOMIC_RELEASE, "wavefront");                                                          \
			__builtin_amdgcn_wave_barrier();                                                                                \
			phase2(cur, i);                                                                                                 \
			__builtin_amdgcn_wave_barrier();                                                                                \
		}
		if (any_bg) {
			GSR_BWQ_WALK(GsBool<true>{})
		} else {
			GSR_BWQ_WALK(GsBool<false>{})
		}
#undef GSR_BWQ_WALK
		thr16 -= GSR_BWQ_BATCH * 16;
#pragma unroll
		for (int qq = 0; qq < 4; qq++) {
			turn_read(qq);
			turn_write(qq);
		}
		TM(9)
		GSR_WAIT_VM0();
		__syncthreads();
		TM(10)
		for (int fj = tid; fj < cnt; fj += GSR_BWD_THREADS) {
			float v[10];
#pragma unroll
			for (int k = 0; k < 10; k++)
				v[k] = ((s_plane[0][fj * GSR_PLANE_STRIDE + k] + s_plane[1][fj * GSR_PLANE_STRIDE + k]) +
				        s_plane[2][fj * GSR_PLANE_STRIDE + k]) + s_plane[3][fj * GSR_PLANE_STRIDE + k];
			const float4 A = sA[fj], B = sB[fj];
			const float ca = -2.f * A.z, cb = -A.w, cc = -2.f * B.x, op = B.y;
			const float M10 = v[0], M01 = v[1], M20 = v[2], M11 = v[3], M02 = v[8];
			const float ddelx_dx = (float)(0.5 * W), ddely_dy = (float)(0.5 * H);
			const uint32_t my_row = s_row[fj];
			float4* dst = reinterpret_cast<float4*>(rows + (size_t)my_row * GSR_ROW_STRIDE);
			dst[0] = make_float4(-(op * FMA(cb, M01, ca * M10)) * ddelx_dx, -(op * FMA(cb, M10, cc * M01)) * ddely_dy,
			                     -0.5f * op * M20, -0.5f * op * M11);
			dst[1] = make_float4(-0.5f * op * M02, v[9], v[4], v[5]);
			dst[2] = make_float4(v[6], v[7], 0.f, 0.f);
			if (FLAGS) row_flags[my_row] = 1;
		}
		TM(11)
	}
	TM_END
}

__global__ void bwd_selftest_kernel(const float* __restrict__ in, uint32_t* __restrict__ out)
{
	const float one = in[0];
	const float r = __builtin_amdgcn_rcpf(one - in[1]);
	uint32_t ok = (__float_as_uint(r) == 0x3f800000u) ? 1u : 0u;
	const float t = 0.37f * in[0];
	if (t * r == t) ok |= 2u;
	out[0] = ok;
	out[1] = __float_as_uint(r);
}
void launch_bwd_selftest(const float* in, uint32_t* out, hipStream_t s)
{
	hipLaunchKernelGGL(bwd_selftest_kernel, dim3(1), dim3(1), 0, s, in, out);
}

__global__ __launch_bounds__(256) void band_classes_kernel(int P, const int* __restrict__ radii, const GsRec* __restrict__ recs, int split,
                                                           int* __restrict__ first, int* __restrict__ second)
{
	const int idx = blockIdx.x * 256 + threadIdx.x;
	if (idx >= P) return;
	const bool vis = radii[idx] > 0;
	const bool c1 = vis && (int)(recs[idx].q3.y >> 16) <= split;
	if (first != nullptr) first[idx] = c1 ? 1 : 0;
	if (second != nullptr) second[idx] = (vis && !c1) ? 1 : 0;
}
void launch_band_classes(int P, const int* radii, const GsRec* recs, int split, int* first, int* second, hipStream_t s)
{
	hipLaunchKernelGGL(band_classes_kernel, dim3((P + 255) / 256), dim3(256), 0, s, P, radii, recs, split, first, second);
}

__device__ __forceinline__ uint32_t gs_work_class(uint32_t m)
{
	if (m < 4u) return m;
	const int e = 31 - __clz((int)m);
	return (uint32_t)(4 * (e - 1)) + ((m >> (e - 2)) & 3u);
}
__global__ __launch_bounds__(256) void tile_work_kernel(int T, const uint32_t* __restrict__ n_contrib, uint32_t* __restrict__ work)
{
	const int tile = blockIdx.x * 4 + (threadIdx.x >> 6), lane = threadIdx.x & 63;
	if (tile >= T) return;
	const uint4 v = reinterpret_cast<const uint4*>(n_contrib + (size_t)tile * GSR_TILE_PIX)[lane];
	uint32_t m = max(max(v.x, v.y), max(v.z, v.w));
#pragma unroll
	for (int o = 32; o > 0; o >>= 1) m = max(m, (uint32_t)__shfl_xor((int)m, o, 64));
	if (lane == 0) work[tile] = m;
}
__global__ __launch_bounds__(1024) void tile_order_kernel(int T, const uint32_t* __restrict__ work, uint32_t* __restrict__ order)
{
	__shared__ uint32_t s_cnt[128], s_cur[128];
	const int tid = threadIdx.x;
	if (tid < 128) s_cnt[tid] = 0u;
	__syncthreads();
	for (int t = tid; t < T; t += 1024) atomicAdd(&s_cnt[gs_work_class(work[t])], 1u);
	__syncthreads();
	if (tid == 0) {
		uint32_t run = 0;
		for (int c = 127; c >= 0; c--) { s_cur[c] = run; run += s_cnt[c]; }
	}
	__syncthreads();
	for (int t = tid; t < T; t += 1024) order[atomicAdd(&s_cur[gs_work_class(work[t])], 1u)] = (uint32_t)t;
}
void launch_tile_order(int T, const uint32_t* n_contrib, uint32_t* tile_work, uint32_t* tile_order, hipStream_t s)
{
	hipLaunchKernelGGL(tile_work_kernel, dim3((T + 3) / 4), dim3(256), 0, s, T, n_contrib, tile_work);
	hipLaunchKernelGGL(tile_order_kernel, dim3(1), dim3(1024), 0, s, T, tile_work, tile_order);
}

void launch_composite_bwd(const ImgLayout& il, int W, int H, const GsBg& bg, const uint2* ranges,
                          const uint32_t* point_list, const GsRec* recs, const uint32_t* goff, const float* final_T,
                          const uint32_t* n_contrib, const uint32_t* med_pos, const float* dL_dpix, const float* dL_dpix_depth,
                          const float* dL_dpix_median, const float* dL_dpix_opacity, float* rows, uint8_t* row_flags,
                          const GsCtl* ctl, int variant, hipStream_t s)
{
	const int tb_n = (int)std::min(bg.tile_hi, (uint32_t)il.T) - (int)bg.tile_lo;
	const int chunk = bg.tile_order ? (il.T + 7) / 8 : std::max(1, (tb_n + 7) / 8);
	const bool tsel = (variant & 1) != 0, wave_lists = (variant & 2) != 0;
	const bool fx = (variant & 8) != 0;
	const bool flags = row_flags != nullptr;
#define GSR_LAUNCH_CB(...)                                                                                         \
	hipLaunchKernelGGL((__VA_ARGS__), dim3(chunk * 8), dim3(GSR_BWD_THREADS), 0, s, il.T, chunk, il.gx, W, H, bg,  \
	                   ranges, point_list, recs, goff, final_T, n_contrib, med_pos, dL_dpix, dL_dpix_depth, dL_dpix_median, \
	                   dL_dpix_opacity, rows, row_flags, ctl)
#ifdef GSR_AB_VARIANTS
	if (wave_lists) {
		if (flags) { if (tsel) GSR_LAUNCH_CB(composite_bwd_kernel<true, true>); else GSR_LAUNCH_CB(composite_bwd_kernel<true, false>); }
		else { if (tsel) GSR_LAUNCH_CB(composite_bwd_kernel<false, true>); else GSR_LAUNCH_CB(composite_bwd_kernel<false, false>); }
	} else
#else
	(void)wave_lists;
#endif
	if (dL_dpix_depth == nullptr && dL_dpix_median == nullptr && dL_dpix_opacity == nullptr && !tsel) {
		if (fx) { if (flags) GSR_LAUNCH_CB(composite_bwd_quarter_kernel<true, false, true, true>); else GSR_LAUNCH_CB(composite_bwd_quarter_kernel<false, false, true, true>); }
		else { if (flags) GSR_LAUNCH_CB(composite_bwd_quarter_kernel<true, false, false, true>); else GSR_LAUNCH_CB(composite_bwd_quarter_kernel<false, false, false, true>); }
	} else if (fx) {
		if (flags) { if (tsel) GSR_LAUNCH_CB(composite_bwd_quarter_kernel<true, true, true, false>); else GSR_LAUNCH_CB(composite_bwd_quarter_kernel<true, false, true, false>); }
		else { if (tsel) GSR_LAUNCH_CB(composite_bwd_quarter_kernel<false, true, true, false>); else GSR_LAUNCH_CB(composite_bwd_quarter_kernel<false, false, true, false>); }
	} else {
		if (flags) { if (tsel) GSR_LAUNCH_CB(composite_bwd_quarter_kernel<true, true, false, false>); else GSR_LAUNCH_CB(composite_bwd_quarter_kernel<true, false, false, false>); }
		else { if (tsel) GSR_LAUNCH_CB(composite_bwd_quarter_kernel<false, true, false, false>); else GSR_LAUNCH_CB(composite_bwd_quarter_kernel<false, false, false, false>); }
	}
#undef GSR_LAUNCH_CB
}

template <int D, bool FLAGS>
__global__ __launch_bounds__(256) void preprocess_bwd_kernel(
    int P, int M, const float* __restrict__ means3D, const int* __restrict__ radii, const float* __restrict__ shs,
    const float* __restrict__ scales, const float* __restrict__ rotations, float scale_modifier,
    const float* __restrict__ cov3D_precomp, const GsCam* __restrict__ cam, int W, int H, float tan_fovx,
    float tan_fovy, float h_x, float h_y, int sh_vec4, int act, const GsRec* __restrict__ recs,
    const uint32_t* __restrict__ goff, const float* __restrict__ rows, const uint8_t* __restrict__ row_flags,
    float* __restrict__ dL_dmean2D, float* __restrict__ dL_dopacity, float* __restrict__ dL_dcolor,
    float* __restrict__ dL_dmeans, float* __restrict__ dL_dcov, float* __restrict__ dL_dsh,
    float* __restrict__ dL_dscale, float* __restrict__ dL_drot, int mask_colors, int cls_mode, int cls_split)
{
	const int idx = blockIdx.x * 256 + threadIdx.x;
	bool mine = true;
	if (cls_mode != 0) {
		const bool v_ = idx < P && radii[idx] > 0;
		const int rmaxy = v_ ? (int)(recs[idx].q3.y >> 16) : 0;
		mine = ((!v_ || rmaxy <= cls_split) ? 1 : 2) == cls_mode;
		if (__ballot(mine && idx < P) == 0ull) return;
	}
	float a_[GSR_ROW_STRIDE];
	{
		__shared__ float4 s_rows[4][GSR_SUM_SLAB * 3];
		__shared__ uint8_t s_flag[4][(GSR_SUM_SLAB + 63) / 64 * 64];
		const int lane = threadIdx.x & 63, wv = threadIdx.x >> 6;
		const int g0 = blockIdx.x * 256 + wv * 64;
		if (g0 >= P) return;
		const uint32_t b = goff[min(idx, P)], e = (idx < P && mine) ? goff[idx + 1] : b;
		const uint32_t wb = goff[g0], we = goff[min(g0 + 64, P)];
		const bool is_long = e - b > (uint32_t)GSR_SUM_LONG;
#pragma unroll
		for (int i = 0; i < GSR_ROW_STRIDE; i++) a_[i] = 0.f;
		float4* slab = s_rows[wv];
		for (uint32_t base = wb; base < we; base += GSR_SUM_SLAB) {
			const uint32_t cnt = min((uint32_t)GSR_SUM_SLAB, we - base);
			const float4* src = reinterpret_cast<const float4*>(rows + (size_t)base * GSR_ROW_STRIDE);
			uint8_t* fl = s_flag[wv];
			constexpr bool flagged = FLAGS;
			if (flagged) {
#pragma unroll
				for (int it = 0; it < (GSR_SUM_SLAB + 63) / 64; it++) {
					const uint32_t r = it * 64 + lane;
					fl[r] = r < cnt ? row_flags[base + r] : (uint8_t)0;
				}
				__builtin_amdgcn_wave_barrier();
			}
#pragma unroll
			for (int it = 0; it < (GSR_SUM_SLAB * 3 + 63) / 64; it++) {
				const uint32_t j = it * 64 + lane;
				if (j < cnt * 3 && (!flagged || fl[j / 3])) slab[j] = gs_ld_stream(src + j);
			}
			__builtin_amdgcn_wave_barrier();
			const uint32_t lo = max(b, base), hi = is_long ? lo : min(e, base + cnt);
			for (uint32_t r = lo; r < hi; r++) {
				if (flagged && !fl[r - base]) continue;
				const float4* ar = slab + (r - base) * 3;
				const float4 v0 = ar[0], v1 = ar[1], v2 = ar[2];
				a_[0] += v0.x; a_[1] += v0.y; a_[2] += v0.z; a_[3] += v0.w; a_[4] += v1.x; a_[5] += v1.y;
				a_[6] += v1.z; a_[7] += v1.w; a_[8] += v2.x; a_[9] += v2.y;
			}
			__builtin_amdgcn_wave_barrier();
		}
// ... 574 lines not shown
```

### gaustudio_amd/csrc/gsr_kernels_fwd.hip

```cpp
#include "gsr_internal.h"

namespace gsr {

__device__ __constant__ float kSH_C0 = 0.28209479177387814f;
__device__ __constant__ float kSH_C1 = 0.4886025119029199f;
__device__ __constant__ float kSH_C2[5] = {1.0925484305920792f, -1.0925484305920792f, 0.31539156525252005f,
                                            -1.0925484305920792f, 0.5462742152960396f};
__device__ __constant__ float kSH_C3[7] = {-0.5900435899266435f, 2.890611442640554f, -0.4570457994644658f,
                                            0.3731763325901154f, -0.4570457994644658f, 1.445305721320277f,
                                            -0.5900435899266435f};

__global__ __launch_bounds__(256) void mark_visible_kernel(int P, const float* __restrict__ means3D,
                                                           const float* __restrict__ view,
                                                           unsigned char* __restrict__ present)
{
	int idx = blockIdx.x * 256 + threadIdx.x;
	if (idx >= P) return;
	float3 p = {means3D[3 * idx], means3D[3 * idx + 1], means3D[3 * idx + 2]};
	float3 pv = xform4x3(p, view);
	present[idx] = !(pv.z <= 0.2f);
}

void launch_mark_visible(int P, const float* means3D, const float* view, unsigned char* present, hipStream_t s)
{
// ... 1408 lines not shown
	}
	const uint32_t nf = min(nfq_, fall_cap);
	for (uint32_t it = blockIdx.x; it < nf; it += gridDim.x) {
		const uint2 sg = fall_items[it];
		const bool in_keys = (sg.y & GSR_Q_IN_KEYS) != 0u;
		gs_radix_sort_segment((in_keys ? keys : keys2) + sg.x, (in_keys ? keys2 : keys) + sg.x, point_list + sg.x, sg.y & ~GSR_Q_IN_KEYS,
		                      whist, s_tot, &s_maxrun);
	}
	const int lane = threadIdx.x & 63;
	const uint32_t nitems = min(nsq_, sort_cap);
	const uint32_t nwaves = gridDim.x * 4u;
	for (uint32_t it = blockIdx.x * 4u + (threadIdx.x >> 6); it < nitems; it += nwaves) {
		const uint2 item = sort_items[it];
		const uint32_t cnt = item.y & ~GSR_Q_IN_KEYS;
		const uint64_t* bs = ((item.y & GSR_Q_IN_KEYS) ? keys : keys2) + item.x;
		uint32_t* bo = point_list + item.x;
		if (cnt <= 64) gs_wave_sort_tile<1>(bs, bo, cnt, lane);
		else if (cnt <= 128) gs_wave_sort_tile<2>(bs, bo, cnt, lane);
		else if (cnt <= 256) gs_wave_sort_tile<4>(bs, bo, cnt, lane);
		else if (cnt <= 512) gs_wave_sort_tile<8>(bs, bo, cnt, lane);
		else gs_wave_sort_tile<16>(bs, bo, cnt, lane);
	}
}

struct SortQueueLayout {
	uint32_t sort_cap, seg_cap, slice_cap;
	size_t sort_items, seg_items, slice_items, rows, total;
	SortQueueLayout(size_t R, int T)
	{
		sort_cap = (uint32_t)(R / 16 + 4 * (size_t)T + 4096);
		seg_cap = (uint32_t)(R / 512 + (size_t)T + 64);
		slice_cap = (uint32_t)(R / GSR_SLICE_KEYS + std::min((size_t)T, R / GSR_SORT_LDS_MAX) + 1);
		sort_items = 256;
		seg_items = sort_items + sizeof(uint2) * (size_t)sort_cap;
		slice_items = (seg_items + sizeof(uint2) * 2 * (size_t)seg_cap + 15) & ~(size_t)15;
		rows = slice_items + sizeof(uint4) * (size_t)slice_cap;
		total = rows + sizeof(uint16_t) * GSR_SLICE_ROW * (size_t)slice_cap + 256;
	}
};
size_t sort_queue_bytes(size_t R, int T) { return SortQueueLayout(R, T).total; }

#ifndef GSR_RADIX_RK_SHORT
#define GSR_RADIX_RK_SHORT 16
#endif
void launch_tile_sort(int T, bool with_short, int long_level, const uint2* ranges, uint64_t* keys, uint64_t* keys2,
                      uint32_t* point_list, char* queue, size_t R, GsCtl* ctl, uint32_t cap, uint32_t* host_err, hipStream_t s)
{
	if (long_level <= 1) {
		if (with_short)
			hipLaunchKernelGGL(tile_sort_kernel, dim3((T + 3) / 4), dim3(256), 0, s, T, ranges, keys, point_list, ctl, cap, (GsSortQ*)nullptr,
			                   (uint4*)nullptr, 0u, (uint64_t*)nullptr);
		if (long_level == 1) {
			hipLaunchKernelGGL(tile_radix_sort_kernel<GSR_RADIX_RK_SHORT>, dim3(T), dim3(256), 0, s, ranges, keys, keys2, point_list, GSR_SORT_LDS_MAX,
			                   256u * GSR_RADIX_RK_SHORT, (GsSortQ*)nullptr, (uint2*)nullptr, 0u, ctl, cap);
			hipLaunchKernelGGL(tile_radix_sort_kernel<32>, dim3(T), dim3(256), 0, s, ranges, keys, keys2, point_list, 256u * GSR_RADIX_RK_SHORT,
			                   0xffffffffu, (GsSortQ*)nullptr, (uint2*)nullptr, 0u, ctl, cap);
		}
		return;
	}
	const SortQueueLayout ql(R, T);
	const uint32_t sort_cap = ql.sort_cap, seg_cap = ql.seg_cap, slice_cap = ql.slice_cap;
	GsSortQ* q = reinterpret_cast<GsSortQ*>(queue);
	uint2* sort_items = reinterpret_cast<uint2*>(queue + ql.sort_items);
	uint2* seg_items = reinterpret_cast<uint2*>(queue + ql.seg_items);
	uint2* fall_items = seg_items + seg_cap;
	uint4* slice_items = reinterpret_cast<uint4*>(queue + ql.slice_items);
	uint16_t* rows = reinterpret_cast<uint16_t*>(queue + ql.rows);
	(void)hipMemsetAsync(q, 0, sizeof(GsSortQ), s);
	hipLaunchKernelGGL(tile_sort_kernel, dim3((T + 3) / 4), dim3(256), 0, s, T, ranges, keys, point_list, ctl, cap, q, slice_items, slice_cap, keys2);
	hipLaunchKernelGGL(tile_radix_sort_kernel<GSR_RADIX_RK_SHORT>, dim3(T), dim3(256), 0, s, ranges, keys, keys2, point_list, GSR_SORT_LDS_MAX,
	                   256u * GSR_RADIX_RK_SHORT, q, seg_items, seg_cap, ctl, cap);
	hipLaunchKernelGGL(tile_radix_sort_kernel<32>, dim3(T), dim3(256), 0, s, ranges, keys, keys2, point_list, 256u * GSR_RADIX_RK_SHORT, 0xffffffffu, q,
	                   seg_items, seg_cap, ctl, cap);
	hipLaunchKernelGGL(slice_hist_kernel, dim3(512), dim3(GSR_PART_THREADS), 0, s, keys, keys2, point_list, q, slice_items, slice_cap, rows, ctl, cap);
	hipLaunchKernelGGL(slice_scatter_kernel, dim3(512), dim3(GSR_PART_THREADS), 0, s, keys, keys2, point_list, q, slice_items, slice_cap, rows,
	                   sort_items, sort_cap, seg_items, seg_cap, ctl, cap);
	hipLaunchKernelGGL(segment_partition_kernel, dim3(128), dim3(GSR_PART_THREADS), 0, s, keys, keys2, q, sort_items, sort_cap,
	                   seg_items, &q->n_seg, seg_cap, fall_items, &q->n_fall, ctl, cap);
	hipLaunchKernelGGL(bucket_sort_kernel, dim3(2048), dim3(256), 0, s, keys, keys2, point_list, q, sort_items, sort_cap, fall_items, seg_cap, ctl, cap,
	                   &ctl->err_overflow, host_err);
}


#ifdef GSR_AB_VARIANTS
template <bool NOCULL>
__global__ __launch_bounds__(256) void composite_fwd_kernel(
    int T, int chunk, int gx, int W, int H, const uint2* __restrict__ ranges,
    const uint32_t* __restrict__ point_list, const GsRec* __restrict__ recs, float* __restrict__ out_color,
    float* __restrict__ out_depth, float* __restrict__ out_median, float* __restrict__ out_opacity,
    float* __restrict__ final_T, uint32_t* __restrict__ n_contrib, uint32_t* __restrict__ med_pos_out,
    const GsCtl* __restrict__ ctl, uint32_t cap, uint32_t max_sorted, const uint32_t* __restrict__ tile_order,
    uint32_t* __restrict__ staged_out)
{
	__shared__ float4 sA[256];
	__shared__ float4 sB[256];
	__shared__ float4 sC[256];
	if (ctl->num_binned > cap || ctl->max_tile_count > max_sorted) return;
	const int tile = tile_order ? ((int)blockIdx.x < T ? (int)tile_order[blockIdx.x] : T) : (blockIdx.x & 7) * chunk + (blockIdx.x >> 3);
	if ((!tile_order && (int)(blockIdx.x >> 3) >= chunk) || tile >= T) return;
	const int tid = threadIdx.x;
	const int lane = tid & 63;
	const int tx = tile % gx, ty = tile / gx;
	int lx, ly;
	gs_pixel_of_thread(tid, lx, ly);
	const int px = tx * GSR_BLOCK_X + lx, py = ty * GSR_BLOCK_Y + ly;
	const bool inside = px < W && py < H;
	const float pixfx = (float)px, pixfy = (float)py;
	const float bx0 = (float)(tx * GSR_BLOCK_X + (((tid >> 6) & 1) << 3));
	const float by0 = (float)(ty * GSR_BLOCK_Y + (((tid >> 6) >> 1) << 3));
	const float bx1 = fminf(bx0 + 7.f, (float)(W - 1)), by1 = fminf(by0 + 7.f, (float)(H - 1));
	const uint2 range = ranges[tile];
	const int total = (int)(range.y - range.x);
	bool done = !inside;
	float T_ = 1.0f;
	uint32_t last_contributor = 0;
	v2f acc01 = {0.f, 0.f}, acc23 = {0.f, 0.f};
	uint32_t med_pos = 0;
	float med_T = 0.f;

	int staged = 0;
	for (int base = 0; base < total; base += 256) {
		if (__syncthreads_and(done)) break;
		const int cnt = min(256, total - base);
		staged += cnt;
		if (tid < cnt) {
			const uint32_t id = point_list[range.x + base + tid];
			const GsRec* r = recs + id;
			sA[tid] = r->q0;
			float4 b = r->q1;
			float4 c = r->q2;
			c.w = b.z;
			b.z = __int_as_float((int)id);
			sB[tid] = b;
			sC[tid] = c;
		}
		__syncthreads();
		for (int sub = 0; sub < cnt; sub += 64) {
			if (__ballot(!done) == 0ull) break;
			const int jl = sub + lane;
			bool hit = false;
			if (jl < cnt) hit = NOCULL ? true : gs_box_may_touch(sA[jl], sB[jl], bx0, by0, bx1, by1);
			unsigned long long m = __ballot(hit);
			while (m) {
				const int j = sub + __ffsll((long long)m) - 1;
				m &= m - 1;
				const float4 A = sA[j], B = sB[j], Cc = sC[j];
				const float dx = A.x - pixfx, dy = A.y - pixfy;
				const float power = FMA(A.w * dx, dy, FMA(B.x * dy, dy, (A.z * dx) * dx));
				const float alpha = fminf(0.99f, B.y * gs_exp(power));
				const bool valid = (!done) & (power <= 0.0f) & (power >= (NOCULL ? -80.0f : B.w)) & (!(alpha < 1.0f / 255.0f));
				const float test_T = T_ * (1 - alpha);
				const bool stop = valid & (test_T < 0.0001f);
				done = done | stop;
				const bool apply = valid & (!stop);
				const float w = apply ? alpha * T_ : 0.f;
				acc01 = vfma(v2f{Cc.x, Cc.y}, v2f{w, w}, acc01);
				acc23 = vfma(v2f{Cc.z, Cc.w}, v2f{w, w}, acc23);
				const bool medc = apply & (T_ > 0.5f);
				med_pos = medc ? (uint32_t)(base + j + 1) : med_pos;
				med_T = medc ? T_ : med_T;
				T_ = apply ? test_T : T_;
				last_contributor = apply ? (uint32_t)(base + j + 1) : last_contributor;
			}
		}
	}
	final_T[(size_t)tile * GSR_TILE_PIX + tid] = T_;
	n_contrib[(size_t)tile * GSR_TILE_PIX + tid] = last_contributor;
	uint32_t med_final = 0;
	if (inside) {
		float median_D = 15.0f, median_weight = 0.f;
		int median_id = 0;
		if (med_pos != 0) {
			const uint32_t id = point_list[range.x + med_pos - 1];
			const GsRec* r = recs + id;
			const float4 A = r->q0, B = r->q1;
			const float dx = A.x - pixfx, dy = A.y - pixfy;
			const float power = FMA(A.w * dx, dy, FMA(B.x * dy, dy, (A.z * dx) * dx));
			const float alpha = fminf(0.99f, B.y * gs_exp(power));
			if (med_T * (1 - alpha) < 0.5f) {
				median_D = B.z;
				median_weight = alpha * med_T;
				median_id = (int)id;
				med_final = med_pos;
			}
		}
		const size_t HW = (size_t)H * W;
		const size_t pix_id = (size_t)W * py + px;
		out_color[pix_id] = acc01.x;
		out_color[HW + pix_id] = acc01.y;
		out_color[2 * HW + pix_id] = acc23.x;
		out_depth[pix_id] = acc23.y;
		out_median[pix_id] = median_D;
		out_median[HW + pix_id] = median_weight;
		out_median[2 * HW + pix_id] = (float)median_id;
		out_opacity[pix_id] = 1 - T_;
	}
	med_pos_out[(size_t)tile * GSR_TILE_PIX + tid] = med_final;
	if (tid == 0 && staged_out != nullptr) staged_out[tile] = (uint32_t)staged;
}

#endif

#define GSR_FWD_PLANE 257
#define GSR_FWD_SENT_OFF (256 * 16)
#define GSR_FWD_LIST 264
#define GSR_FWD_NONE 0xffffu

#ifndef GSR_FWD_MED_SPLIT
#define GSR_FWD_MED_SPLIT 1
#endif
#ifndef GSR_FWD_WAVES
#define GSR_FWD_WAVES 7
#endif
template <bool NOCULL, bool FX>
__global__ __launch_bounds__(256) __attribute__((amdgpu_waves_per_eu(GSR_FWD_WAVES, GSR_FWD_WAVES))) void composite_fwd_quarter_kernel(
    int T, int chunk, int gx, int W, int H, const uint2* __restrict__ ranges,
    const uint32_t* __restrict__ point_list, const GsRec* __restrict__ recs, float* __restrict__ out_color,
    float* __restrict__ out_depth, float* __restrict__ out_median, float* __restrict__ out_opacity,
    float* __restrict__ final_T, uint32_t* __restrict__ n_contrib, uint32_t* __restrict__ med_pos_out,
    GsCtl* __restrict__ ctl, uint32_t cap, uint32_t max_sorted, const uint32_t* __restrict__ tile_order,
    uint32_t* __restrict__ staged_out)
{
	__shared__ float4 sRec[3 * GSR_FWD_PLANE];
	__shared__ uint16_t sMask[256];
	__shared__ __attribute__((aligned(16))) uint16_t sList[4][4][GSR_FWD_LIST];
	const uint32_t num_binned = ctl->num_binned;
	if (num_binned > cap || ctl->max_tile_count > max_sorted) return;
	uint16_t* __restrict__ qmask = gs_qmask_ptr(point_list, num_binned);
	if (!NOCULL && blockIdx.x == 0 && threadIdx.x == 0) ctl->has_qmask = 1u;
	if (FX && blockIdx.x == 0 && threadIdx.x == 0) ctl->opts |= GSR_CTL_OPT_FAST_EXP;
	const int tile = tile_order ? ((int)blockIdx.x < T ? (int)tile_order[blockIdx.x] : T) : (blockIdx.x & 7) * chunk + (blockIdx.x >> 3);
	if ((!tile_order && (int)(blockIdx.x >> 3) >= chunk) || tile >= T) return;
	const int tid = threadIdx.x;
	const int lane = tid & 63, w = tid >> 6, q = lane >> 4;
	const int tx = tile % gx, ty = tile / gx;
	const int lx = ((w & 1) << 3) + ((q & 1) << 2) + (lane & 3);
	const int ly = ((w >> 1) << 3) + ((q >> 1) << 2) + ((lane >> 2) & 3);
	const int slot = (w << 6) + ((ly & 7) << 3) + (lx & 7);
	const int px = tx * GSR_BLOCK_X + lx, py = ty * GSR_BLOCK_Y + ly;
	const bool inside = px < W && py < H;
	const float pixfx = (float)px, pixfy = (float)py;
	const float tx0 = (float)(tx * GSR_BLOCK_X), ty0 = (float)(ty * GSR_BLOCK_Y);
	uint32_t allq = 0;
#pragma unroll
	for (int b = 0; b < 16; b++)
		if (tx * GSR_BLOCK_X + 4 * (b & 3) < W && ty * GSR_BLOCK_Y + 4 * (b >> 2) < H) allq |= 1u << b;
	const uint2 range = ranges[tile];
	const int total = (int)(range.y - range.x);
	bool done = !inside;
	float T_ = 1.0f;
	uint32_t last_contributor = 0;
	v2f acc01 = {0.f, 0.f}, acc23 = {0.f, 0.f};
	uint32_t med_pos = 0;
	float med_T = 0.f;
#if GSR_FWD_MED_SPLIT
	bool med_live = true;
#endif
	if (tid < 3) sRec[tid * GSR_FWD_PLANE + 256] = make_float4(0.f, 0.f, 0.f, 0.f);
	const char* rec_base = reinterpret_cast<const char*>(sRec);
	const uint16_t* my_list = &sList[w][q][0];

	int staged = 0;
	for (int base = 0; base < total; base += 256) {
		if (__syncthreads_and(done)) break;
		const int cnt = min(256, total - base);
		staged += cnt;
		uint32_t mk = 0;
		if (tid < cnt) {
			const uint32_t id = point_list[range.x + base + tid];
			const GsRec* rr = recs + id;
			const float4 a = rr->q0;
			float4 b = rr->q1;
			float4 c = rr->q2;
			mk = NOCULL ? allq : gs_quarter_mask<4>(a, b, tx0, ty0, allq);
			if (!NOCULL) qmask[range.x + base + tid] = (uint16_t)mk;
			c.w = b.z;
			b.z = __int_as_float((int)id);
			sRec[tid] = a;
			sRec[GSR_FWD_PLANE + tid] = b;
			sRec[2 * GSR_FWD_PLANE + tid] = c;
		}
		sMask[tid] = (uint16_t)mk;
		{
			uint4* l4 = reinterpret_cast<uint4*>(&sList[w][0][0]);
			const uint32_t ss = GSR_FWD_SENT_OFF | (GSR_FWD_SENT_OFF << 16);
			for (int k = lane; k < 4 * GSR_FWD_LIST / 8; k += 64) l4[k] = make_uint4(ss, ss, ss, ss);
		}
		__syncthreads();
		int c0 = 0, c1 = 0, c2 = 0, c3 = 0;
		const int wbit = 8 * (w >> 1) + 2 * (w & 1);
		for (int sub = 0; sub < cnt; sub += 64) {
			const uint32_t m16 = (uint32_t)sMask[sub + lane] >> wbit;
			const uint32_t off = (uint32_t)(sub + lane) << 4;
#define GSR_APPEND(QQ, SH, CNT)                                                                          \
	{                                                                                                    \
		const bool h = (m16 >> (SH)) & 1u;                                                               \
		const unsigned long long bm = __ballot(h);                                                       \
		const int pos = CNT + (int)__builtin_amdgcn_mbcnt_hi((uint32_t)(bm >> 32), __builtin_amdgcn_mbcnt_lo((uint32_t)bm, 0u)); \
		if (h) sList[w][QQ][pos] = (uint16_t)off;                                                        \
		CNT += __popcll(bm);                                                                             \
	}
			GSR_APPEND(0, 0, c0)
// ... 13 lines not shown
		__builtin_amdgcn_sched_barrier(0);                                                                                   \
		_Pragma("unroll") for (int k = 0; k < 4; k++) {                                                                      \
			const uint32_t off = offs[k];                                                                                    \
			const float4 A = *reinterpret_cast<const float4*>(rec_base + off);                                               \
			const float4 B = *reinterpret_cast<const float4*>(rec_base + off + GSR_FWD_PLANE * 16);                          \
			const float4 Cc = *reinterpret_cast<const float4*>(rec_base + off + 2 * GSR_FWD_PLANE * 16);                     \
			const float dx = A.x - pixfx, dy = A.y - pixfy;                                                                  \
			const float power = FMA(A.w * dx, dy, FMA(B.x * dy, dy, (A.z * dx) * dx));                                      \
			const float alpha = fminf(0.99f, B.y * (FX ? gs_exp_hw(power) : gs_exp(power)));                                 \
			const bool valid = (!done) & (power <= 0.0f) & (FX ? true : (power >= (NOCULL ? -80.0f : B.w))) &                \
			                   (!(alpha < 1.0f / 255.0f));                                                                   \
			const float test_T = T_ * (1 - alpha);                                                                           \
			const bool stop = valid & (test_T < 0.0001f);                                                                    \
			done = done | stop;                                                                                              \
			const bool apply = valid & (!stop);                                                                              \
			const float wgt = apply ? alpha * T_ : 0.f;                                                                      \
			acc01 = vfma(v2f{Cc.x, Cc.y}, v2f{wgt, wgt}, acc01);                                                             \
			acc23 = vfma(v2f{Cc.z, Cc.w}, v2f{wgt, wgt}, acc23);                                                             \
			if (MED) {                                                                                                       \
				const bool medc = apply & (T_ > 0.5f);                                                                       \
				med_off = medc ? off : med_off;                                                                              \
				med_T = medc ? T_ : med_T;                                                                                   \
			}                                                                                                                \
			T_ = apply ? test_T : T_;                                                                                        \
			last_off = apply ? off : last_off;                                                                               \
		}                                                                                                                    \
	}
#if GSR_FWD_MED_SPLIT
		int i = 0;
		if (med_live) {
			for (; i < n; i += 4) {
				if (__builtin_amdgcn_ballot_w64((!done) & (T_ > 0.5f)) == 0ull) { med_live = false; break; }
				GSR_FWD_GROUP(true)
			}
		}
		if (!med_live && __builtin_amdgcn_ballot_w64(!done) != 0ull) {
			for (; i < n; i += 4) {
				if ((i & 31) == 0 && __ballot(!done) == 0ull) break;
				GSR_FWD_GROUP(false)
			}
		}
#else
		for (int i = 0; i < n; i += 4) {
			if ((i & 31) == 0 && __ballot(!done) == 0ull) break;
			GSR_FWD_GROUP(true)
		}
#endif
#undef GSR_FWD_GROUP
		if (last_off != GSR_FWD_NONE) last_contributor = (uint32_t)base + (last_off >> 4) + 1u;
		if (med_off != GSR_FWD_NONE) med_pos = (uint32_t)base + (med_off >> 4) + 1u;
	}
	final_T[(size_t)tile * GSR_TILE_PIX + slot] = T_;
	n_contrib[(size_t)tile * GSR_TILE_PIX + slot] = last_contributor;
	uint32_t med_final = 0;
	if (inside) {
		float median_D = 15.0f, median_weight = 0.f;
		int median_id = 0;
		if (med_pos != 0) {
			const uint32_t id = point_list[range.x + med_pos - 1];
			const GsRec* rr = recs + id;
			const float4 A = rr->q0, B = rr->q1;
			const float dx = A.x - pixfx, dy = A.y - pixfy;
			const float power = FMA(A.w * dx, dy, FMA(B.x * dy, dy, (A.z * dx) * dx));
			const float alpha = fminf(0.99f, B.y * (FX ? gs_exp_hw(power) : gs_exp(power)));
			if (med_T * (1 - alpha) < 0.5f) {
				median_D = B.z;
				median_weight = alpha * med_T;
				median_id = (int)id;
				med_final = med_pos;
			}
		}
		const size_t HW = (size_t)H * W;
		const size_t pix_id = (size_t)W * py + px;
		out_color[pix_id] = acc01.x;
		out_color[HW + pix_id] = acc01.y;
		out_color[2 * HW + pix_id] = acc23.x;
		out_depth[pix_id] = acc23.y;
		out_median[pix_id] = median_D;
		out_median[HW + pix_id] = median_weight;
		out_median[2 * HW + pix_id] = (float)median_id;
		out_opacity[pix_id] = 1 - T_;
	}
	med_pos_out[(size_t)tile * GSR_TILE_PIX + slot] = med_final;
	if (tid == 0 && staged_out != nullptr) staged_out[tile] = (uint32_t)staged;
}

__device__ __forceinline__ uint32_t gs_len_class(uint32_t m)
{
	if (m < 4u) return m;
	const int e = 31 - __clz((int)m);
	return (uint32_t)(4 * (e - 1)) + ((m >> (e - 2)) & 3u);
}
__global__ __launch_bounds__(1024) void tile_order_fwd_kernel(int T, const uint2* __restrict__ ranges, uint32_t* __restrict__ order,
                                                             const GsCtl* __restrict__ ctl, uint32_t cap)
{
	__shared__ uint32_t s_cnt[128], s_cur[128];
	if (ctl->num_binned > cap) return;
	const int tid = threadIdx.x;
	if (tid < 128) s_cnt[tid] = 0u;
	__syncthreads();
	for (int t = tid; t < T; t += 1024) atomicAdd(&s_cnt[gs_len_class(ranges[t].y - ranges[t].x)], 1u);
	__syncthreads();
	if (tid == 0) {
		uint32_t run = 0;
		for (int c = 127; c >= 0; c--) { s_cur[c] = run; run += s_cnt[c]; }
	}
	__syncthreads();
	for (int t = tid; t < T; t += 1024) order[atomicAdd(&s_cur[gs_len_class(ranges[t].y - ranges[t].x)], 1u)] = (uint32_t)t;
}
void launch_tile_order_fwd(int T, const uint2* ranges, uint32_t* order, const GsCtl* ctl, uint32_t cap, hipStream_t s)
{
	hipLaunchKernelGGL(tile_order_fwd_kernel, dim3(1), dim3(1024), 0, s, T, ranges, order, ctl, cap);
}

void launch_composite_fwd(const ImgLayout& il, int W, int H, const uint2* ranges, const uint32_t* point_list,
                          const GsRec* recs, float* out_color, float* out_depth, float* out_median,
                          float* out_opacity, float* final_T, uint32_t* n_contrib, uint32_t* med_pos,
                          GsCtl* ctl_, uint32_t cap, uint32_t max_sorted, bool nocull, bool wave_lists, bool fast_exp,
                          const uint32_t* tile_order, uint32_t* staged_out, hipStream_t s)
{
	const int chunk = (il.T + 7) / 8;
#define GSR_LAUNCH_FWD(K)                                                                                              \
	hipLaunchKernelGGL(K, dim3(chunk * 8), dim3(256), 0, s, il.T, chunk, il.gx, W, H, ranges, point_list, recs, out_color, \
	                   out_depth, out_median, out_opacity, final_T, n_contrib, med_pos, ctl, cap, max_sorted, tile_order, staged_out)
#ifdef GSR_AB_VARIANTS
	if (wave_lists) {
		const GsCtl* ctl = ctl_;
		if (nocull) GSR_LAUNCH_FWD(composite_fwd_kernel<true>);
		else GSR_LAUNCH_FWD(composite_fwd_kernel<false>);
	} else
#endif
	{
		GsCtl* ctl = ctl_;
		if (fast_exp) {
			if (nocull) GSR_LAUNCH_FWD((composite_fwd_quarter_kernel<true, true>));
			else GSR_LAUNCH_FWD((composite_fwd_quarter_kernel<false, true>));
		} else {
			if (nocull) GSR_LAUNCH_FWD((composite_fwd_quarter_kernel<true, false>));
			else GSR_LAUNCH_FWD((composite_fwd_quarter_kernel<false, false>));
		}
	}
#undef GSR_LAUNCH_FWD
}

}
```

### include/gsrast.h

```cpp
#ifndef GSRAST_H_INCLUDED
#define GSRAST_H_INCLUDED

#include <stddef.h>
#include <stdint.h>

#ifdef __cplusplus
extern "C" {
#endif

#define GSR_OK 0
#define GSR_ERR_HIP (-1)
#define GSR_ERR_ARG (-2)
#define GSR_ERR_PREFILTERED (-3)
#define GSR_ERR_ALLOC (-4)
#define GSR_ERR_NONFINITE (-5)
#define GSR_ERR_NONFINITE_QUERY (-6)

typedef char* (*gsr_alloc_fn)(void* ctx, size_t bytes);

int gsr_abi_version(void);

const char* gsr_last_error(void);

int gsr_mark_visible(int P, const float* means3D, const float* viewmatrix, const float* projmatrix,
// ... 93 lines not shown
int gsr_pack_geometry(int P, const uint32_t* hdr, const float* g_means3D, const float* g_opacity, const float* g_scales,
                      const float* g_rotations, float* rows, uint32_t* flag_outside, void* stream);
int gsr_unpack_geometry(int P, const uint32_t* hdr, const float* rows, float* g_means3D, float* g_opacity, float* g_scales,
                        float* g_rotations, void* stream);
int gsr_sh_grad_from_packed(int P, int D, int M, int N, const float* means3D, const float* campos, const uint32_t* msgs,
                            const unsigned long long* msg_offsets, float* dL_dsh, void* stream);

int gsr_set_option(const char* name, int value);
int gsr_get_option(const char* name);

typedef struct gsr_options {
	int32_t struct_bytes;
	int32_t tight_binning;
	int32_t cull;
	int32_t fwd_variant;
	int32_t bwd_variant;
	int32_t speculative;
	int32_t tile_row_lo;
	int32_t tile_row_hi;
	int32_t fast_exp;
	int32_t forward_only;
} gsr_options;
void gsr_options_init(gsr_options* opt);

int gsr_forward_ex(const gsr_options* opt, gsr_alloc_fn geometry_alloc, void* geometry_ctx, gsr_alloc_fn binning_alloc,
                   void* binning_ctx, gsr_alloc_fn image_alloc, void* image_ctx, int P, int D, int M,
                   const float* background, int width, int height, const float* means3D, const float* shs,
                   const float* shs_rest, const float* colors_precomp, const float* opacities, const float* scales,
                   float scale_modifier, const float* rotations, const float* cov3D_precomp, int activation_flags,
                   const float* viewmatrix, const float* projmatrix, const float* cam_pos, float tan_fovx, float tan_fovy,
                   int prefiltered, float* out_color, float* out_depth, float* out_median_depth, float* out_opacity,
                   int* radii, int debug, void* stream);
int gsr_backward_ex(const gsr_options* opt, int parts, int sh_g0, int sh_g1, int P, int D, int M, int R,
                    const float* background, int width, int height, const float* means3D, const float* shs,
                    const float* shs_rest, const float* colors_precomp, const float* scales, float scale_modifier,
                    const float* rotations, const float* cov3D_precomp, int activation_flags, float tan_fovx,
                    float tan_fovy, const int* radii, const char* geom_buffer, const char* binning_buffer,
                    const char* image_buffer, const float* dL_dpix, const float* dL_dpix_depth,
                    const float* dL_dpix_median_depth, const float* dL_dpix_final_opacity, float* dL_dmean2D,
                    float* dL_dopacity, float* dL_dcolor, float* dL_dmean3D, float* dL_dcov3D, float* dL_dsh,
                    float* dL_dsh_rest, float* dL_dscale, float* dL_drot, char* scratch, int debug, void* stream);

int gsr_selftest(void* stream);

#define GSR_ACT_OPACITY_SIGMOID 1
#define GSR_ACT_SCALE_EXP 2
#define GSR_ACT_ROT_NORMALIZE 4

int gsr_forward_raw(gsr_alloc_fn geometry_alloc, void* geometry_ctx, gsr_alloc_fn binning_alloc, void* binning_ctx,
                    gsr_alloc_fn image_alloc, void* image_ctx, int P, int D, int M, const float* background, int width,
                    int height, const float* means3D, const float* f_dc, const float* f_rest, const float* raw_opacities,
                    const float* raw_scales, float scale_modifier, const float* raw_rotations, int activation_flags,
                    const float* viewmatrix, const float* projmatrix, const float* cam_pos, float tan_fovx,
                    float tan_fovy, int prefiltered, float* out_color, float* out_depth, float* out_median_depth,
                    float* out_opacity, int* radii, int debug, void* stream);

int gsr_backward_raw(int P, int D, int M, int R, const float* background, int width, int height, const float* means3D,
                     const float* f_dc, const float* f_rest, const float* raw_scales, float scale_modifier,
                     const float* raw_rotations, int activation_flags, float tan_fovx, float tan_fovy,
                     const int* radii, const char* geom_buffer, const char* binning_buffer, const char* image_buffer,
                     const float* dL_dpix, const float* dL_dpix_depth, const float* dL_dpix_median_depth,
                     const float* dL_dpix_final_opacity, float* dL_dmean2D, float* dL_draw_opacity, float* dL_dcolor,
                     float* dL_dmean3D, float* dL_dcov3D, float* dL_df_dc, float* dL_df_rest, float* dL_draw_scale,
                     float* dL_draw_rot, char* scratch, int debug, void* stream);


int gsr_inspect_geometry(const char* geom_buffer, int P, const int* radii, float* means2D, float* depths,
                         float* conic_opacity, float* rgb, unsigned char* clamped,
                         uint32_t* tiles_touched, void* stream);

int gsr_inspect_backward_sums(const char* geom_buffer, const char* scratch, int P, int R, const int* radii,
                               float* sums, void* stream);

int gsr_inspect_counts(const char* image_buffer, int width, int height, uint32_t out[4], void* stream);

int gsr_inspect_staged(const char* image_buffer, int width, int height, unsigned long long* staged_total, void* stream);

int gsr_inspect_binning(const char* binning_buffer, const char* image_buffer, int R, int width, int height,
                        uint32_t* point_list, uint32_t* ranges, void* stream);

int gsr_inspect_image(const char* image_buffer, int width, int height, float* final_T,
                      uint32_t* n_contrib, void* stream);


int gsr_depth_to_points(const float* depth, int width, int height, const float* intrinsics,
                        const float* world_to_camera, float* points, void* stream);

int gsr_depth_to_normals(const float* depth, int width, int height, const float* intrinsics, int k, float d_min,
                         float d_max, const float* world_to_camera, float* normals, void* stream);
int gsr_depth_epilogue(const float* depth, const float* opacity, float min_opacity, int width, int height,
                       const float* intrinsics, int k, float d_min, float d_max, const float* world_to_camera, float* points,
                       float* normals, void* stream);

int gsr_masked_bilateral(const float* depth, const unsigned char* mask, int width, int height, int d, float sigma_color,
                         float sigma_space, float* filtered, unsigned char* new_mask, unsigned int* scratch2, void* stream);


int gsr_tsdf_integrate(const float* points, int num_points, const float origin[3], float voxel_size, float sdf_trunc,
                       int space_carving, uint64_t* block_keys, uint64_t capacity, uint64_t* voxels, uint32_t* status,
                       void* stream);
int gsr_tsdf_integrate_map(const float* points, int num_points, int row_width, const float origin[3], float voxel_size,
                           float sdf_trunc, int space_carving, uint64_t* block_keys, uint64_t capacity, uint64_t* voxels,
                           uint32_t* status, void* stream);

int gsr_tsdf_export_blocks(const uint64_t* voxels, const uint32_t* block_slots, int num_blocks, float sdf_trunc,
                           uint32_t* counts, float* tsdf, int64_t* sums, void* stream);

int gsr_tsdf_mc_classify(const uint64_t* block_keys, uint64_t capacity, const uint64_t* voxels, const uint32_t* block_slots,
                         int num_blocks, const uint32_t* slot_to_block, float sdf_trunc, float min_weight, int fill_holes,
                         uint8_t* cases, uint32_t* edge_flags, uint32_t* block_num_vertices, uint32_t* block_num_triangles,
                         void* stream);
int gsr_tsdf_mc_emit(const uint64_t* block_keys, uint64_t capacity, const uint64_t* voxels, const uint32_t* block_slots,
                     int num_blocks, const uint32_t* slot_to_block, float voxel_size, float sdf_trunc, const uint8_t* cases,
                     const uint32_t* edge_flags, const uint32_t* block_vertex_offset, const uint32_t* block_triangle_offset,
                     uint32_t* vertex_base, float* vertices, int* triangles, void* stream);


int gsr_ctsdf_touch(const float* depth, int width, int height, int stride, const float intrinsic[4], const float cam_to_world[12],
                    float depth_trunc, float voxel_length, float sdf_trunc, uint64_t* block_keys, uint64_t capacity,
                    int* slot_stamp, int frame, uint32_t* status, int lane_filter, uint64_t* counters, void* stream);
int gsr_ctsdf_integrate(const float* depth, const void* color, int color_mode, int width, int height, const float intrinsic[4],
                        const float world_to_cam[12], float depth_trunc, float voxel_length, float sdf_trunc,
                        const uint64_t* block_keys, const int* touched_slots, int num_touched, float* voxels, void* stream);
int gsr_ctsdf_export_blocks(const float* voxels, const uint32_t* block_slots, int num_blocks, float* tsdf, float* weight, float* color,
                            void* stream);
int gsr_ctsdf_mc_classify(const uint64_t* block_keys, uint64_t capacity, const float* voxels, const uint32_t* block_slots, int num_blocks,
                          const uint32_t* slot_to_block, float min_weight, uint8_t* cases, uint32_t* edge_flags,
                          uint32_t* block_num_vertices, uint32_t* block_num_triangles, void* stream);
int gsr_ctsdf_mc_emit(const uint64_t* block_keys, uint64_t capacity, const float* voxels, const uint32_t* block_slots, int num_blocks,
                      const uint32_t* slot_to_block, float voxel_length, const uint8_t* cases, const uint32_t* edge_flags,
                      const uint32_t* block_vertex_offset, const uint32_t* block_triangle_offset, uint32_t* vertex_base, float* vertices,
                      float* colors, int* triangles, void* stream);

int gsr_surfel_forward(const gsr_options* opt, gsr_alloc_fn geometry_alloc, void* geometry_ctx, gsr_alloc_fn binning_alloc,
                       void* binning_ctx, gsr_alloc_fn image_alloc, void* image_ctx, int P, int D, int M, const float* background,
                       int width, int height, const float* means3D, const float* shs, const float* colors_precomp,
                       const float* opacities, const float* scales, float scale_modifier, const float* rotations,
                       const float* viewmatrix, const float* projmatrix, const float* cam_pos, float* out_color, float* out_allmap,
                       int* radii, int debug, void* stream);
size_t gsr_surfel_scratch_bytes(int P, int R);
int gsr_surfel_backward(const gsr_options* opt, int P, int D, int M, int R, int width, int height, const float* means3D,
                        const float* shs, const float* colors_precomp, const float* scales, float scale_modifier,
                        const float* rotations, const int* radii, const char* geom_buffer, const char* binning_buffer,
                        const char* image_buffer, const float* out_color, const float* out_allmap, const float* dL_dout_color,
                        const float* dL_dout_allmap, float* dL_dmean2D, float* dL_dopacity, float* dL_dcolor, float* dL_dmean3D,
                        float* dL_dsh, float* dL_dscale, float* dL_drot, char* scratch, int debug, void* stream);

#define GSR_KNN_MAX_K 64

int gsr_knn(gsr_alloc_fn workspace_alloc, void* workspace_ctx, const float* points, int num_points, const float* queries,
            int num_queries, int k, double* dist2, int64_t* indices, void* stream);

int gsr_fusion_records(const float* xyz, int num_gaussians, const int* ids, const float* normals, const float* confidences,
                       int num_records, const float w2c_translation[3], int* records, int* status, void* stream);

int gsr_fusion_group(gsr_alloc_fn workspace_alloc, void* workspace_ctx, const int* records, int num_records, int num_gaussians,
                     float consistency, int* unique_ids, float* mean_normals, void* stream);

int gsr_fusion_smooth(gsr_alloc_fn workspace_alloc, void* workspace_ctx, const float* xyz, const int* unique_ids,
                      const float* mean_normals, int num_unique, int k, float sigma, float* normals, void* stream);

int gsr_outlier_statistical(gsr_alloc_fn workspace_alloc, void* workspace_ctx, const float* points, int num_points,
                            int nb_neighbors, double std_ratio, unsigned char* keep, double* mean_distance, void* stream);

int gsr_outlier_normal(gsr_alloc_fn workspace_alloc, void* workspace_ctx, const float* points, const double* normals,
                       int num_points, int nb_neighbors, double angle_threshold, unsigned char* keep, void* stream);
// ... 158 lines not shown
```

Baseline: 2314 Mpixels/s.

## Record per-wave contributor bounds in forward; use them in backward and tile ordering

The forward composite kernel now reduces each wave's last-contributor count with DPP ops and stores a per-tile uint4 bound. The backward kernel reads this bound up front instead of reducing n_contrib across waves through shared memory and a __syncthreads. That lets it issue the first record and gradient loads before the block barrier, and exit early, after zeroing rows, for tiles with no contributors. The tile ordering pass drops its separate reduction kernel and reads the stored bounds directly. In exchange the forward pass does a small reduction and store per wave, some loads are made unconditional with clamped indices, and a new inspect API is added.

New measurement: 2325 Mpixels/s (median of 6 runs). No clear change (+0.5%).

```diff
diff --git a/__graft_entry__.py b/__graft_entry__.py
--- a/__graft_entry__.py
+++ b/__graft_entry__.py
@@ -21,7 +21,7 @@
     for sym in ("gsr_forward", "gsr_backward", "gsr_mark_visible", "gsr_backward_scratch_bytes", "gsr_last_error",
                 "gsr_inspect_geometry", "gsr_inspect_binning", "gsr_inspect_image", "gsr_inspect_backward_sums", "gsr_set_profiling",
                 "gsr_last_forward_ms", "gsr_last_backward_ms", "gsr_forward_raw", "gsr_backward_raw", "gsr_forward_ex", "gsr_backward_ex", "gsr_options_init", "gsr_depth_to_points",
-                "gsr_depth_to_normals", "gsr_depth_epilogue", "gsr_backward_parts", "gsr_set_option", "gsr_get_option", "gsr_selftest", "gsr_inspect_counts", "gsr_inspect_staged", "gsr_tsdf_integrate", "gsr_tsdf_integrate_map", "gsr_tsdf_export_blocks", "gsr_tsdf_mc_classify", "gsr_tsdf_mc_emit", "gsr_msg_header_words", "gsr_visible_index", "gsr_union_index", "gsr_pack_rows", "gsr_unpack_rows", "gsr_pack_geometry", "gsr_unpack_geometry",
+                "gsr_depth_to_normals", "gsr_depth_epilogue", "gsr_backward_parts", "gsr_set_option", "gsr_get_option", "gsr_selftest", "gsr_inspect_counts", "gsr_inspect_staged", "gsr_inspect_tile_bound", "gsr_tsdf_integrate", "gsr_tsdf_integrate_map", "gsr_tsdf_export_blocks", "gsr_tsdf_mc_classify", "gsr_tsdf_mc_emit", "gsr_msg_header_words", "gsr_visible_index", "gsr_union_index", "gsr_pack_rows", "gsr_unpack_rows", "gsr_pack_geometry", "gsr_unpack_geometry",
                 "gsr_sh_grad_from_packed", "gsr_band_classes", "gsr_mesh_rasterize", "gsr_mesh_interpolate",
                 "gsr_mesh_vertex_normals", "gsr_mesh_visible_faces", "gsr_psr_rasterize", "gsr_psr_spectral", "gsr_psr_interp",
                 "gsr_psr_normalize", "gsr_psr_mc_classify", "gsr_psr_mc_emit", "gsr_psr_mc_normals", "gsr_psr_rasterize_bwd",
diff --git a/gaustudio_amd/_C.py b/gaustudio_amd/_C.py
--- a/gaustudio_amd/_C.py
+++ b/gaustudio_amd/_C.py
@@ -215,6 +215,13 @@
     return final_T, n_contrib
 
 
+def inspect_tile_bound(imgBuffer, width, height):
+    T = ((width + 15) // 16) * ((height + 15) // 16)
+    words = torch.empty((T, 4), dtype=torch.int32, device=imgBuffer.device)
+    _call("gsr_inspect_tile_bound", imgBuffer.device, imgBuffer, int(width), int(height), words)
+    return words
+
+
 def set_profiling(enable):
     lib().gsr_set_profiling(ctypes.c_int(int(enable)))
 
diff --git a/gaustudio_amd/csrc/gsr_api.hip b/gaustudio_amd/csrc/gsr_api.hip
--- a/gaustudio_amd/csrc/gsr_api.hip
+++ b/gaustudio_amd/csrc/gsr_api.hip
@@ -523,6 +523,7 @@
 	float* final_T = reinterpret_cast<float*>(img + il.final_T);
 	uint32_t* n_contrib = reinterpret_cast<uint32_t*>(img + il.n_contrib);
 	uint32_t* med_pos = reinterpret_cast<uint32_t*>(img + il.med_pos);
+	uint4* tile_bound = reinterpret_cast<uint4*>(img + il.tile_bound);
 
 	Timer tm(prof_next(g_fwd_log), s, kFwdStages, g_prof_fwd_mask);
 	static_assert(sizeof(GsCtl) == 8 * sizeof(uint32_t), "stage_cam_kernel clears GsCtl word by word");
@@ -612,7 +613,7 @@
 			order = o;
 		}
 		launch_composite_fwd(il, width, height, ranges, point_list, recs, out_color, out_depth, out_median_depth,
-		                     out_opacity, final_T, n_contrib, med_pos, ctl, cap,
+		                     out_opacity, final_T, n_contrib, med_pos, tile_bound, ctl, cap,
 		                     long_level >= 2 ? 0xffffffffu : (long_level == 1 ? GSR_SORT_GIANT : GSR_SORT_LDS_MAX), nocull, wave_lists, ro.fast_exp != 0, order,
 		                     tile_count , s);
 		STAGE_CHECK("composite_fwd", debug, s);
@@ -761,6 +762,7 @@
 	const float* final_T = reinterpret_cast<const float*>(image_buffer + il.final_T);
 	const uint32_t* n_contrib = reinterpret_cast<const uint32_t*>(image_buffer + il.n_contrib);
 	const uint32_t* med_pos = reinterpret_cast<const uint32_t*>(image_buffer + il.med_pos);
+	const uint4* tile_bound = reinterpret_cast<const uint4*>(image_buffer + il.tile_bound);
 	const uint32_t* point_list = reinterpret_cast<const uint32_t*>(binning_buffer + bl.point_list);
 	const BwdLayout wl((size_t)P, (size_t)(R > 0 ? R : 0));
 	const uint32_t* goff = reinterpret_cast<const uint32_t*>(geom_buffer + gl.goff);
@@ -860,12 +862,11 @@
 			variant |= 8;
 		}
 		if (fwd.skew) {
-			uint32_t* tw = reinterpret_cast<uint32_t*>(const_cast<char*>(image_buffer) + il.tile_work);
 			uint32_t* to = reinterpret_cast<uint32_t*>(const_cast<char*>(image_buffer) + il.tile_order);
-			launch_tile_order(il.T, n_contrib, tw, to, s);
+			launch_tile_order(il.T, tile_bound, to, s);
 			bgv.tile_order = to;
 		}
-		launch_composite_bwd(il, width, height, bgv, ranges, point_list, recs, goff, final_T, n_contrib, med_pos, dL_dpix,
+		launch_composite_bwd(il, width, height, bgv, ranges, point_list, recs, goff, final_T, n_contrib, med_pos, tile_bound, dL_dpix,
 		                     dL_dpix_depth, dL_dpix_median_depth, dL_dpix_final_opacity, rows, row_flags,
 		                     reinterpret_cast<const GsCtl*>(image_buffer + il.ctl), variant, s);
 		STAGE_CHECK("composite_bwd", debug, s);
@@ -1166,6 +1167,16 @@
 	                   reinterpret_cast<const float*>(image_buffer + il.final_T),
 	                   reinterpret_cast<const uint32_t*>(image_buffer + il.n_contrib), final_T, n_contrib);
 	STAGE_CHECK("inspect_image", 0, s);
+	return GSR_OK;
+}
+
+int gsr_inspect_tile_bound(const char* image_buffer, int width, int height, uint32_t* bound_words, void* stream)
+{
+	hipStream_t s = (hipStream_t)stream;
+	g_err.clear();
+	if (!image_buffer || !bound_words) return fail(GSR_ERR_ARG, "gsr_inspect_tile_bound: NULL argument", __FILE__, __LINE__);
+	const ImgLayout il(width, height);
+	HIP_TRY(hipMemcpyAsync(bound_words, image_buffer + il.tile_bound, sizeof(uint4) * (size_t)il.T, hipMemcpyDeviceToDevice, s));
 	return GSR_OK;
 }
 
diff --git a/gaustudio_amd/csrc/gsr_internal.h b/gaustudio_amd/csrc/gsr_internal.h
--- a/gaustudio_amd/csrc/gsr_internal.h
+++ b/gaustudio_amd/csrc/gsr_internal.h
@@ -26,7 +26,7 @@
 };
 
 struct ImgLayout {
-	size_t ctl, ranges, tile_count, final_T, n_contrib, med_pos, tile_work, tile_order, total;
+	size_t ctl, ranges, tile_count, final_T, n_contrib, med_pos, tile_bound, tile_order, total;
 	int gx, gy, T;
 	ImgLayout(int W, int H)
 	{
@@ -39,8 +39,8 @@
 		final_T = tile_count + align_up(sizeof(uint32_t) * (size_t)T);
 		n_contrib = final_T + align_up(sizeof(float) * (size_t)T * GSR_TILE_PIX);
 		med_pos = n_contrib + align_up(sizeof(uint32_t) * (size_t)T * GSR_TILE_PIX);
-		tile_work = med_pos + align_up(sizeof(uint32_t) * (size_t)T * GSR_TILE_PIX);
-		tile_order = tile_work + align_up(sizeof(uint32_t) * (size_t)T);
+		tile_bound = med_pos + align_up(sizeof(uint32_t) * (size_t)T * GSR_TILE_PIX);
+		tile_order = tile_bound + align_up(sizeof(uint4) * (size_t)T);
 		total = tile_order + align_up(sizeof(uint32_t) * (size_t)T);
 	}
 };
@@ -104,7 +104,7 @@
                       uint32_t* point_list, char* queue, size_t R, GsCtl* ctl, uint32_t cap, uint32_t* host_err, hipStream_t s);
 void launch_composite_fwd(const ImgLayout& il, int W, int H, const uint2* ranges, const uint32_t* point_list,
                           const GsRec* recs, float* out_color, float* out_depth, float* out_median,
-                          float* out_opacity, float* final_T, uint32_t* n_contrib, uint32_t* med_pos, GsCtl* ctl, uint32_t cap, uint32_t max_sorted, bool nocull, bool wave_lists, bool fast_exp,
+                          float* out_opacity, float* final_T, uint32_t* n_contrib, uint32_t* med_pos, uint4* tile_bound, GsCtl* ctl, uint32_t cap, uint32_t max_sorted, bool nocull, bool wave_lists, bool fast_exp,
                           const uint32_t* tile_order, uint32_t* staged_out, hipStream_t s);
 void launch_tile_order_fwd(int T, const uint2* ranges, uint32_t* order, const GsCtl* ctl, uint32_t cap, hipStream_t s);
 
@@ -148,10 +148,10 @@
 	uint32_t tile_lo, tile_hi;
 };
 void launch_band_classes(int P, const int* radii, const GsRec* recs, int split, int* first, int* second, hipStream_t s);
-void launch_tile_order(int T, const uint32_t* n_contrib, uint32_t* tile_work, uint32_t* tile_order, hipStream_t s);
+void launch_tile_order(int T, const uint4* tile_bound, uint32_t* tile_order, hipStream_t s);
 void launch_composite_bwd(const ImgLayout& il, int W, int H, const GsBg& bg, const uint2* ranges,
                           const uint32_t* point_list, const GsRec* recs, const uint32_t* goff, const float* final_T,
-                          const uint32_t* n_contrib, const uint32_t* med_pos, const float* dL_dpix, const float* dL_dpix_depth,
+                          const uint32_t* n_contrib, const uint32_t* med_pos, const uint4* tile_bound, const float* dL_dpix, const float* dL_dpix_depth,
                           const float* dL_dpix_median, const float* dL_dpix_opacity, float* rows, uint8_t* row_flags,
                           const GsCtl* ctl, int variant, hipStream_t s);
 #define GSR_PART_GEOM 1
diff --git a/gaustudio_amd/csrc/gsr_kernels_bwd.hip b/gaustudio_amd/csrc/gsr_kernels_bwd.hip
--- a/gaustudio_amd/csrc/gsr_kernels_bwd.hip
+++ b/gaustudio_amd/csrc/gsr_kernels_bwd.hip
@@ -161,7 +161,7 @@
     int T, int chunk, int gx, int W, int H, const GsBg bgv, const uint2* __restrict__ ranges,
     const uint32_t* __restrict__ point_list, const GsRec* __restrict__ recs, const uint32_t* __restrict__ goff,
     const float* __restrict__ final_T, const uint32_t* __restrict__ n_contrib, const uint32_t* __restrict__ med_pos,
-    const float* __restrict__ dL_dpix, const float* __restrict__ dL_dpix_depth, const float* __restrict__ dL_dpix_median,
+    const uint4* __restrict__ tile_bound, const float* __restrict__ dL_dpix, const float* __restrict__ dL_dpix_depth, const float* __restrict__ dL_dpix_median,
     const float* __restrict__ dL_dpix_opacity, float* __restrict__ rows, uint8_t* __restrict__ row_flags,
     const GsCtl* __restrict__ ctl)
 {
@@ -383,7 +383,7 @@
     int T, int chunk, int gx, int W, int H, const GsBg bgv, const uint2* __restrict__ ranges,
     const uint32_t* __restrict__ point_list, const GsRec* __restrict__ recs, const uint32_t* __restrict__ goff,
     const float* __restrict__ final_T, const uint32_t* __restrict__ n_contrib, const uint32_t* __restrict__ med_pos,
-    const float* __restrict__ dL_dpix, const float* __restrict__ dL_dpix_depth, const float* __restrict__ dL_dpix_median,
+    const uint4* __restrict__ tile_bound, const float* __restrict__ dL_dpix, const float* __restrict__ dL_dpix_depth, const float* __restrict__ dL_dpix_median,
     const float* __restrict__ dL_dpix_opacity, float* __restrict__ rows, uint8_t* __restrict__ row_flags,
     const GsCtl* __restrict__ ctl)
 {
@@ -395,7 +395,6 @@
 	__shared__ __attribute__((aligned(16))) float s_plane[4][GSR_BWQ_BATCH * GSR_PLANE_STRIDE];
 	__shared__ __attribute__((aligned(16))) float2 s_slab[4][4 * GSR_BWQ_QSTRIDE];
 	__shared__ __attribute__((aligned(16))) uint16_t s_list[4][4][GSR_BWQ_LIST];
-	__shared__ int s_max[4];
 	if (blockIdx.x == 0 && threadIdx.x == 0 && bgv.flag_dst != nullptr) *bgv.flag_dst = bgv.flag;
 	const int tb_lo = (int)bgv.tile_lo, tb_n = (int)min(bgv.tile_hi, (uint32_t)T) - tb_lo;
 	const int local = (blockIdx.x & 7) * chunk + (blockIdx.x >> 3);
@@ -413,28 +412,79 @@
 	const float pixfx = (float)px, pixfy = (float)py;
 	const float fbx = (float)(tx * GSR_BLOCK_X + ((wv & 1) << 3)), fby = (float)(ty * GSR_BLOCK_Y + ((wv >> 1) << 3));
 	const uint2 range = ranges[tile];
+	const uint4 tb4 = tile_bound[tile];
+	const int bmax = (int)max(max(tb4.x, tb4.y), max(tb4.z, tb4.w));
 	const bool have_qmask = __builtin_amdgcn_readfirstlane(ctl->has_qmask) != 0u;
 	const uint16_t* __restrict__ qmask = gs_qmask_ptr(point_list, __builtin_amdgcn_readfirstlane(ctl->num_binned));
 
+	const int srec = tid >> 2, spart = tid & 3;
+	const uint32_t* __restrict__ tile_list = point_list + range.x;
+	const uint32_t* __restrict__ mask_words = have_qmask ? reinterpret_cast<const uint32_t*>(qmask) : point_list;
+	auto list_pos = [&](int t, int h) -> uint32_t {
+		return (uint32_t)max(t - 1 - (srec + 64 * h), 0);
+	};
+	auto word_ptr = [&](int t, int h, uint32_t id) -> const uint32_t* {
+		return spart == 2 ? mask_words + ((range.x + list_pos(t, h)) >> 1) : goff + id;
+	};
+	auto zero_rows = [&](int from) {
+		for (int i = from + tid; !FLAGS && i < (int)(range.y - range.x); i += GSR_BWD_THREADS) {
+			const uint32_t id = tile_list[i];
+			const uint4 q3 = recs[id].q3;
+			float4* dst = reinterpret_cast<float4*>(rows + (size_t)(goff[id] + gs_row_in_rect(q3.x, q3.y, (q3.z >> GSR_Q3Z_DEAD_SHIFT) & 15u, tx, ty)) * GSR_ROW_STRIDE);
+			dst[0] = make_float4(0.f, 0.f, 0.f, 0.f);
+			dst[1] = make_float4(0.f, 0.f, 0.f, 0.f);
+			dst[2] = make_float4(0.f, 0.f, 0.f, 0.f);
+		}
+	};
+	if (bmax <= 0) {
+		zero_rows(0);
+		return;
+	}
+	uint32_t id_cur[GSR_BWQ_HALVES], id_next[GSR_BWQ_HALVES];
+	float4 part[GSR_BWQ_HALVES];
+#pragma unroll
+	for (int h = 0; h < GSR_BWQ_HALVES; h++) {
+		id_cur[h] = tile_list[list_pos(bmax, h)];
+		id_next[h] = tile_list[list_pos(bmax - GSR_BWQ_BATCH, h)];
+	}
+
 	const size_t sidx = (size_t)tile * GSR_TILE_PIX + (wv << 6) + ((ly & 7) << 3) + (lx & 7);
-	const float T_final = inside ? final_T[sidx] : 0.f;
-	const int lc = inside ? (int)n_contrib[sidx] : 0;
-	float dLp0 = 0.f, dLp1 = 0.f, dLp2 = 0.f, dLd = 0.f, dLo = 0.f, dLm = 0.f;
+	float T_final = final_T[sidx];
+	int lc = (int)n_contrib[sidx];
+	float dLp0, dLp1, dLp2, dLd = 0.f, dLo = 0.f, dLm = 0.f;
 	uint32_t mpos = 0u;
-	if (inside) {
+	{
 		const size_t HW = (size_t)H * W;
-		const size_t pix_id = (size_t)W * py + px;
-		if (dL_dpix) {
-			dLp0 = dL_dpix[pix_id];
-			dLp1 = dL_dpix[HW + pix_id];
-			dLp2 = dL_dpix[2 * HW + pix_id];
-		}
+		const size_t pix_id = (size_t)W * min(py, H - 1) + min(px, W - 1);
+		auto grad_at = [&](const float* g, size_t plane_off) -> float {
+			const float v = (g ? g + plane_off : final_T)[pix_id];
+			return g ? v : 0.f;
+		};
+		dLp0 = grad_at(dL_dpix, 0);
+		dLp1 = grad_at(dL_dpix, HW);
+		dLp2 = grad_at(dL_dpix, 2 * HW);
 		if (!CONLY) {
-			if (dL_dpix_depth) dLd = dL_dpix_depth[pix_id];
-			if (dL_dpix_median) dLm = dL_dpix_median[pix_id];
-			if (dL_dpix_opacity) dLo = dL_dpix_opacity[pix_id];
+			dLd = grad_at(dL_dpix_depth, 0);
+			dLm = grad_at(dL_dpix_median, 0);
+			dLo = grad_at(dL_dpix_opacity, 0);
 			mpos = med_pos[sidx];
 		}
+	}
+	const float* __restrict__ bgp = bgv.dptr ? bgv.dptr : final_T;
+	const float bgd0 = bgp[0], bgd1 = bgp[1], bgd2 = bgp[2];
+#pragma unroll
+	for (int h = 0; h < GSR_BWQ_HALVES; h++) {
+		const float4* rp = reinterpret_cast<const float4*>(recs + id_cur[h]) + spart;
+		const uint32_t* wp = spart >= 2 ? word_ptr(bmax, h, id_cur[h]) : reinterpret_cast<const uint32_t*>(rp) + 3;
+		part[h] = *rp;
+		part[h].w = __uint_as_float(*wp);
+	}
+	TM(0)
+	if (!inside) {
+		T_final = 0.f;
+		lc = 0;
+		dLp0 = dLp1 = dLp2 = dLd = dLo = dLm = 0.f;
+		mpos = 0u;
 	}
 	float2* slab = s_slab[wv];
 	float* plane = s_plane[wv];
@@ -461,7 +511,7 @@
 		for (int sx = 0; sx < 4; sx++) asm volatile("" : "+v"(g_pix[sx].x), "+v"(g_pix[sx].y), "+v"(g_pix[sx].z), "+v"(g_pix[sx].w));
 	}
 	const float y2 = fby + (float)(((qd >> 1) << 2) + r2), x2 = fbx + (float)((qd & 1) << 2);
-	const float bg0 = bgv.dptr ? bgv.dptr[0] : bgv.host[0], bg1 = bgv.dptr ? bgv.dptr[1] : bgv.host[1], bg2 = bgv.dptr ? bgv.dptr[2] : bgv.host[2];
+	const float bg0 = bgv.dptr ? bgd0 : bgv.host[0], bg1 = bgv.dptr ? bgd1 : bgv.host[1], bg2 = bgv.dptr ? bgd2 : bgv.host[2];
 	const float bg_dot = FMA(bg2, dLp2, FMA(bg1, dLp1, FMA(bg0, dLp0, 0.f)));
 	const bool any_bg = __ballot(bg_dot != 0.f) != 0ull;
 	float T_ = T_final;
@@ -474,51 +524,10 @@
 	qmax = max(qmax, __shfl_xor(qmax, 8, 64));
 	const int qm0 = __builtin_amdgcn_readlane(qmax, 0), qm1 = __builtin_amdgcn_readlane(qmax, 16);
 	const int qm2 = __builtin_amdgcn_readlane(qmax, 32), qm3 = __builtin_amdgcn_readlane(qmax, 48);
-	const int wmax = max(max(qm0, qm1), max(qm2, qm3));
-	if (lane == 0) s_max[wv] = wmax;
-	TM(0)
 	if (tid < 3) (tid == 0 ? sA : tid == 1 ? sB : sC)[GSR_BWQ_SENT] = make_float4(0.f, 0.f, 0.f, 0.f);
-	__syncthreads();
-	const int bmax = max(max(s_max[0], s_max[1]), max(s_max[2], s_max[3]));
 	TM(1)
 
-	const int srec = tid >> 2, spart = tid & 3;
-	const uint32_t* __restrict__ tile_list = point_list + range.x;
-	const uint32_t* __restrict__ mask_words = have_qmask ? reinterpret_cast<const uint32_t*>(qmask) : point_list;
-	auto list_pos = [&](int t, int h) -> uint32_t {
-		return (uint32_t)max(t - 1 - (srec + 64 * h), 0);
-	};
-	auto word_ptr = [&](int t, int h, uint32_t id) -> const uint32_t* {
-		return spart == 2 ? mask_words + ((range.x + list_pos(t, h)) >> 1) : goff + id;
-	};
-	uint32_t id_next[GSR_BWQ_HALVES];
-	float4 part[GSR_BWQ_HALVES];
-#pragma unroll
-	for (int h = 0; h < GSR_BWQ_HALVES; h++) {
-		part[h] = make_float4(0.f, 0.f, 0.f, 0.f);
-		id_next[h] = 0u;
-	}
-	if (bmax > 0) {
-		uint32_t id_cur[GSR_BWQ_HALVES];
-#pragma unroll
-		for (int h = 0; h < GSR_BWQ_HALVES; h++) {
-			id_cur[h] = tile_list[list_pos(bmax, h)];
-			id_next[h] = tile_list[list_pos(bmax - GSR_BWQ_BATCH, h)];
-		}
-#pragma unroll
-		for (int h = 0; h < GSR_BWQ_HALVES; h++) {
-			part[h] = reinterpret_cast<const float4*>(recs + id_cur[h])[spart];
-			if (spart >= 2) part[h].w = __uint_as_float(*word_ptr(bmax, h, id_cur[h]));
-		}
-	}
-	for (int i = bmax + tid; !FLAGS && i < (int)(range.y - range.x); i += GSR_BWD_THREADS) {
-		const uint32_t id = tile_list[i];
-		const uint4 q3 = recs[id].q3;
-		float4* dst = reinterpret_cast<float4*>(rows + (size_t)(goff[id] + gs_row_in_rect(q3.x, q3.y, (q3.z >> GSR_Q3Z_DEAD_SHIFT) & 15u, tx, ty)) * GSR_ROW_STRIDE);
-		dst[0] = make_float4(0.f, 0.f, 0.f, 0.f);
-		dst[1] = make_float4(0.f, 0.f, 0.f, 0.f);
-		dst[2] = make_float4(0.f, 0.f, 0.f, 0.f);
-	}
+	zero_rows(bmax);
 	GSR_WAIT_VM0();
 	TM(2)
 	const uint16_t* my_list = &s_list[wv][qd][0];
@@ -596,7 +605,9 @@
 				} else {
 					float4 q1 = sB[jl];
 					q1.w = sC[jl].z;
-					mk = gs_quarter_mask<2>(sA[jl], q1, fbx, fby, 0xfu);
+					int ibx = tx * GSR_BLOCK_X + ((wv & 1) << 3), iby = ty * GSR_BLOCK_Y + ((wv >> 1) << 3);
+					asm volatile("" : "+s"(ibx), "+s"(iby));
+					mk = gs_quarter_mask<2>(sA[jl], q1, (float)ibx, (float)iby, 0xfu);
 				}
 				const int pos = top - 1 - jl;
 				mk &= (pos < qm0 ? 1u : 0u) | (pos < qm1 ? 2u : 0u) | (pos < qm2 ? 4u : 0u) | (pos < qm3 ? 8u : 0u);
@@ -806,40 +817,33 @@
 	const int e = 31 - __clz((int)m);
 	return (uint32_t)(4 * (e - 1)) + ((m >> (e - 2)) & 3u);
 }
-__global__ __launch_bounds__(256) void tile_work_kernel(int T, const uint32_t* __restrict__ n_contrib, uint32_t* __restrict__ work)
-{
-	const int tile = blockIdx.x * 4 + (threadIdx.x >> 6), lane = threadIdx.x & 63;
-	if (tile >= T) return;
-	const uint4 v = reinterpret_cast<const uint4*>(n_contrib + (size_t)tile * GSR_TILE_PIX)[lane];
-	uint32_t m = max(max(v.x, v.y), max(v.z, v.w));
-#pragma unroll
-	for (int o = 32; o > 0; o >>= 1) m = max(m, (uint32_t)__shfl_xor((int)m, o, 64));
-	if (lane == 0) work[tile] = m;
-}
-__global__ __launch_bounds__(1024) void tile_order_kernel(int T, const uint32_t* __restrict__ work, uint32_t* __restrict__ order)
+__global__ __launch_bounds__(1024) void tile_order_kernel(int T, const uint4* __restrict__ tile_bound, uint32_t* __restrict__ order)
 {
 	__shared__ uint32_t s_cnt[128], s_cur[128];
 	const int tid = threadIdx.x;
+	auto work = [&](int t) -> uint32_t {
+		const uint4 b = tile_bound[t];
+		return max(max(b.x, b.y), max(b.z, b.w));
+	};
 	if (tid < 128) s_cnt[tid] = 0u;
 	__syncthreads();
-	for (int t = tid; t < T; t += 1024) atomicAdd(&s_cnt[gs_work_class(work[t])], 1u);
+	for (int t = tid; t < T; t += 1024) atomicAdd(&s_cnt[gs_work_class(work(t))], 1u);
 	__syncthreads();
 	if (tid == 0) {
 		uint32_t run = 0;
 		for (int c = 127; c >= 0; c--) { s_cur[c] = run; run += s_cnt[c]; }
 	}
 	__syncthreads();
-	for (int t = tid; t < T; t += 1024) order[atomicAdd(&s_cur[gs_work_class(work[t])], 1u)] = (uint32_t)t;
-}
-void launch_tile_order(int T, const uint32_t* n_contrib, uint32_t* tile_work, uint32_t* tile_order, hipStream_t s)
-{
-	hipLaunchKernelGGL(tile_work_kernel, dim3((T + 3) / 4), dim3(256), 0, s, T, n_contrib, tile_work);
-	hipLaunchKernelGGL(tile_order_kernel, dim3(1), dim3(1024), 0, s, T, tile_work, tile_order);
+	for (int t = tid; t < T; t += 1024) order[atomicAdd(&s_cur[gs_work_class(work(t))], 1u)] = (uint32_t)t;
+}
+void launch_tile_order(int T, const uint4* tile_bound, uint32_t* tile_order, hipStream_t s)
+{
+	hipLaunchKernelGGL(tile_order_kernel, dim3(1), dim3(1024), 0, s, T, tile_bound, tile_order);
 }
 
 void launch_composite_bwd(const ImgLayout& il, int W, int H, const GsBg& bg, const uint2* ranges,
                           const uint32_t* point_list, const GsRec* recs, const uint32_t* goff, const float* final_T,
-                          const uint32_t* n_contrib, const uint32_t* med_pos, const float* dL_dpix, const float* dL_dpix_depth,
+                          const uint32_t* n_contrib, const uint32_t* med_pos, const uint4* tile_bound, const float* dL_dpix, const float* dL_dpix_depth,
                           const float* dL_dpix_median, const float* dL_dpix_opacity, float* rows, uint8_t* row_flags,
                           const GsCtl* ctl, int variant, hipStream_t s)
 {
@@ -850,7 +854,7 @@
 	const bool flags = row_flags != nullptr;
 #define GSR_LAUNCH_CB(...)                                                                                         \
 	hipLaunchKernelGGL((__VA_ARGS__), dim3(chunk * 8), dim3(GSR_BWD_THREADS), 0, s, il.T, chunk, il.gx, W, H, bg,  \
-	                   ranges, point_list, recs, goff, final_T, n_contrib, med_pos, dL_dpix, dL_dpix_depth, dL_dpix_median, \
+	                   ranges, point_list, recs, goff, final_T, n_contrib, med_pos, tile_bound, dL_dpix, dL_dpix_depth, dL_dpix_median, \
 	                   dL_dpix_opacity, rows, row_flags, ctl)
 #ifdef GSR_AB_VARIANTS
 	if (wave_lists) {
diff --git a/gaustudio_amd/csrc/gsr_kernels_fwd.hip b/gaustudio_amd/csrc/gsr_kernels_fwd.hip
--- a/gaustudio_amd/csrc/gsr_kernels_fwd.hip
+++ b/gaustudio_amd/csrc/gsr_kernels_fwd.hip
@@ -1514,13 +1514,25 @@
 }
 
 
+
+__device__ __forceinline__ void gs_store_wave_bound(uint4* __restrict__ tile_bound, int tile, int tid, uint32_t last_contributor)
+{
+	int m = (int)last_contributor;
+	m = max(m, __builtin_amdgcn_update_dpp(0, m, 0xB1, 0xF, 0xF, true));
+	m = max(m, __builtin_amdgcn_update_dpp(0, m, 0x4E, 0xF, 0xF, true));
+	m = max(m, __builtin_amdgcn_update_dpp(0, m, 0x141, 0xF, 0xF, true));
+	m = max(m, __builtin_amdgcn_update_dpp(0, m, 0x140, 0xF, 0xF, true));
+	const int wmax = max(max(__builtin_amdgcn_readlane(m, 0), __builtin_amdgcn_readlane(m, 16)),
+	                     max(__builtin_amdgcn_readlane(m, 32), __builtin_amdgcn_readlane(m, 48)));
+	if ((tid & 63) == 0) reinterpret_cast<uint32_t*>(tile_bound + tile)[tid >> 6] = (uint32_t)wmax;
+}
 #ifdef GSR_AB_VARIANTS
 template <bool NOCULL>
 __global__ __launch_bounds__(256) void composite_fwd_kernel(
     int T, int chunk, int gx, int W, int H, const uint2* __restrict__ ranges,
     const uint32_t* __restrict__ point_list, const GsRec* __restrict__ recs, float* __restrict__ out_color,
     float* __restrict__ out_depth, float* __restrict__ out_median, float* __restrict__ out_opacity,
-    float* __restrict__ final_T, uint32_t* __restrict__ n_contrib, uint32_t* __restrict__ med_pos_out,
+    float* __restrict__ final_T, uint32_t* __restrict__ n_contrib, uint32_t* __restrict__ med_pos_out, uint4* __restrict__ tile_bound,
     const GsCtl* __restrict__ ctl, uint32_t cap, uint32_t max_sorted, const uint32_t* __restrict__ tile_order,
     uint32_t* __restrict__ staged_out)
 {
@@ -1628,6 +1640,7 @@
 		out_opacity[pix_id] = 1 - T_;
 	}
 	med_pos_out[(size_t)tile * GSR_TILE_PIX + tid] = med_final;
+	gs_store_wave_bound(tile_bound, tile, tid, last_contributor);
 	if (tid == 0 && staged_out != nullptr) staged_out[tile] = (uint32_t)staged;
 }
 
@@ -1649,7 +1662,7 @@
     int T, int chunk, int gx, int W, int H, const uint2* __restrict__ ranges,
     const uint32_t* __restrict__ point_list, const GsRec* __restrict__ recs, float* __restrict__ out_color,
     float* __restrict__ out_depth, float* __restrict__ out_median, float* __restrict__ out_opacity,
-    float* __restrict__ final_T, uint32_t* __restrict__ n_contrib, uint32_t* __restrict__ med_pos_out,
+    float* __restrict__ final_T, uint32_t* __restrict__ n_contrib, uint32_t* __restrict__ med_pos_out, uint4* __restrict__ tile_bound,
     GsCtl* __restrict__ ctl, uint32_t cap, uint32_t max_sorted, const uint32_t* __restrict__ tile_order,
     uint32_t* __restrict__ staged_out)
 {
@@ -1829,6 +1842,7 @@
 		out_opacity[pix_id] = 1 - T_;
 	}
 	med_pos_out[(size_t)tile * GSR_TILE_PIX + slot] = med_final;
+	gs_store_wave_bound(tile_bound, tile, tid, last_contributor);
 	if (tid == 0 && staged_out != nullptr) staged_out[tile] = (uint32_t)staged;
 }
 
@@ -1862,14 +1876,14 @@
 
 void launch_composite_fwd(const ImgLayout& il, int W, int H, const uint2* ranges, const uint32_t* point_list,
                           const GsRec* recs, float* out_color, float* out_depth, float* out_median,
-                          float* out_opacity, float* final_T, uint32_t* n_contrib, uint32_t* med_pos,
+                          float* out_opacity, float* final_T, uint32_t* n_contrib, uint32_t* med_pos, uint4* tile_bound,
                           GsCtl* ctl_, uint32_t cap, uint32_t max_sorted, bool nocull, bool wave_lists, bool fast_exp,
                           const uint32_t* tile_order, uint32_t* staged_out, hipStream_t s)
 {
 	const int chunk = (il.T + 7) / 8;
 #define GSR_LAUNCH_FWD(K)                                                                                              \
 	hipLaunchKernelGGL(K, dim3(chunk * 8), dim3(256), 0, s, il.T, chunk, il.gx, W, H, ranges, point_list, recs, out_color, \
-	                   out_depth, out_median, out_opacity, final_T, n_contrib, med_pos, ctl, cap, max_sorted, tile_order, staged_out)
+	                   out_depth, out_median, out_opacity, final_T, n_contrib, med_pos, tile_bound, ctl, cap, max_sorted, tile_order, staged_out)
 #ifdef GSR_AB_VARIANTS
 	if (wave_lists) {
 		const GsCtl* ctl = ctl_;
diff --git a/include/gsrast.h b/include/gsrast.h
--- a/include/gsrast.h
+++ b/include/gsrast.h
@@ -199,6 +199,8 @@
 int gsr_inspect_image(const char* image_buffer, int width, int height, float* final_T,
                       uint32_t* n_contrib, void* stream);
 
+int gsr_inspect_tile_bound(const char* image_buffer, int width, int height, uint32_t* bound_words, void* stream);
+
 
 int gsr_depth_to_points(const float* depth, int width, int height, const float* intrinsics,
                         const float* world_to_camera, float* points, void* stream);
```
